# lh3/miniwfa

Hardware: AMD Instinct MI355X
Metric: aligned Gbp/s (q+t) (higher is better)
Workload: dtype int16x2 packed, range-guarded (bit-exact to the reference's int32); 1 GPU; 1024 pairs/GPU x 10000 bp, 0.05 divergence, score-only mwf_wfa_exact, default penalties (BASELINE configs[2]); pairs_this_gpu=1024, pairs_total=1024, target_len=10000, bases_this_gpu=20479492, grid=512, block=512

## Files before the change

### miniwfa_amd/build.py

```python
from __future__ import annotations

import os
import subprocess
import sys

HERE = os.path.dirname(os.path.abspath(__file__))
ROOT = os.path.dirname(HERE)
CSRC = os.path.join(HERE, "csrc")
LIB = os.path.join(CSRC, "libmwf_hip.so")
SOURCES = ["mwf_band2.hip", "mwf_band2_tab.hip", "mwf_band2_nib.hip", "mwf_band2_e3.hip", "mwf_band2_e4.hip", "mwf_band2_bi.hip", "mwf_band2_bi_deep.hip", "mwf_kernels.hip", "mwf_sketch.hip", "mwf_ends.hip", "mwf_lane.hip", "mwf_mid.hip", "mwf_sys.hip", "mwf_sys_deep.hip", "mwf_cigar_ops.hip", "mwf_cigar_text.hip", "mwf_alphabet.hip", "mwf_engine.cpp", "mwf_memory.cpp", "mwf_plan.cpp", "mwf_chain.cpp", "mwf_async.cpp", "kalloc.cpp", "mwf_dbg.cpp"]
HEADERS = [os.path.join(CSRC, "mwf_internal.h"), os.path.join(CSRC, "mwf_device.h"), os.path.join(CSRC, "mwf_ends.h"), os.path.join(CSRC, "mwf_sys_pass.h"), os.path.join(CSRC, "mwf_band2_kernel.h"), os.path.join(CSRC, "mwf_band2_dispatch.h"), os.path.join(CSRC, "mwf_engine.h"), os.path.join(CSRC, "mwf_plan_classes.h"), os.path.join(CSRC, "mwf_plan_retry.h"), os.path.join(ROOT, "include", "miniwfa.h"), os.path.join(ROOT, "include", "kalloc.h")]
BAND2_UNITS = [s for s in SOURCES if s.startswith("mwf_band2")]


def hipcc() -> str:
    for cand in (os.environ.get("HIPCC"), "/opt/rocm/bin/hipcc", "hipcc"):
        if cand and (os.path.isabs(cand) and os.path.exists(cand) or not os.path.isabs(cand)):
            return cand
    return "hipcc"


def stale() -> bool:
    if not os.path.exists(LIB):
        return True
    t = os.path.getmtime(LIB)
    deps = [os.path.join(CSRC, s) for s in SOURCES if os.path.exists(os.path.join(CSRC, s))] + HEADERS + [os.path.abspath(__file__)]
    return any(os.path.getmtime(d) > t for d in deps)


def build(force: bool = False, verbose: bool = False) -> str:
    if not force and not stale():
        return LIB
    from concurrent.futures import ThreadPoolExecutor
    objdir = os.path.join(CSRC, "build")
    os.makedirs(objdir, exist_ok=True)
    flags = ["--offload-arch=gfx950", "-O3", "-std=c++17", "-fPIC", "-Wall", "-Wno-unused-function", "-I", os.path.join(ROOT, "include"), "-I", CSRC]
    hdr_time = max(os.path.getmtime(h) for h in HEADERS + [os.path.abspath(__file__)])
    jobs, objs = [], []
    for name in SOURCES:
        src = os.path.join(CSRC, name)
        if not os.path.exists(src):
            continue
        obj = os.path.join(objdir, name + ".o")
        objs.append(obj)
        if force or not os.path.exists(obj) or os.path.getmtime(obj) < max(os.path.getmtime(src), hdr_time):
            jobs.append([hipcc(), *flags, "-c", src, "-o", obj])

    def run(cmd):
        if verbose:
            print(" ".join(cmd))
        return cmd, subprocess.run(cmd, capture_output=True, text=True)

    with ThreadPoolExecutor(max(1, min(8, len(jobs)))) as ex:
        for cmd, r in ex.map(run, jobs):
            if r.returncode != 0:
                sys.stderr.write(r.stdout + r.stderr)
                raise RuntimeError("hipcc failed: " + " ".join(cmd))
            if verbose and r.stderr.strip():
                sys.stderr.write(r.stderr)
    cmd, r = run([hipcc(), "--offload-arch=gfx950", "-fPIC", "-shared", *objs, "-o", LIB + ".tmp", "-lpthread"])
    if r.returncode != 0:
        sys.stderr.write(r.stdout + r.stderr)
        raise RuntimeError("hipcc failed linking libmwf_hip.so")
    os.replace(LIB + ".tmp", LIB)
    return LIB


KERNEL_FILES = {"wfa_band2_kernel": "mwf_band2_kernel.h", "wfa_band2_tab_kernel": "mwf_band2_kernel.h", "wfa_band2_nib_kernel": "mwf_band2_kernel.h", "wfa_sys_kernel": "mwf_sys.hip", "wfa_sys_seg_kernel": "mwf_sys.hip",
                "wfa_batch_kernel": "mwf_kernels.hip", "wfa_lane_kernel": "mwf_lane.hip", "wfa_mid_kernel": "mwf_mid.hip", "wfa_ends_kernel": "mwf_ends.hip"}
KERNEL_HEADERS = {"mwf_sys.hip": ["mwf_sys_pass.h", "mwf_sys_deep.hip"], "mwf_band2_kernel.h": ["mwf_band2_dispatch.h", *BAND2_UNITS]}


def kernel_fingerprint(symbol: str) -> str | None:
    import hashlib
    name = symbol.split("<")[0].strip()
    f = KERNEL_FILES.get(name)
    if f is None:
        return None
    h = hashlib.sha256()
    for p in [os.path.join(CSRC, x) for x in [f, *KERNEL_HEADERS.get(f, []), "mwf_device.h", "mwf_internal.h"]]:
        try:
            h.update(open(p, "rb").read())
        except OSError:
            return None
    return h.hexdigest()[:16]


CLI = os.path.join(ROOT, "tools", "test-mwf")


def build_cli(force: bool = False) -> str:
    src = os.path.join(ROOT, "tools", "test-mwf.cpp")
    if not force and os.path.exists(CLI) and os.path.getmtime(CLI) >= max(os.path.getmtime(src), os.path.getmtime(LIB)):
        return CLI
    zl = ["-DMWF_HAVE_ZLIB", "-lz"] if os.path.exists("/usr/include/zlib.h") else []
    cmd = ["g++", "-O2", "-std=c++17", "-Wall", "-I", os.path.join(ROOT, "include"), src, "-o", CLI,
           "-L", CSRC, "-lmwf_hip", "-Wl,-rpath," + CSRC] + zl
    r = subprocess.run(cmd, capture_output=True, text=True)
    if r.returncode != 0:
        sys.stderr.write(r.stdout + r.stderr)
        raise RuntimeError("g++ failed building tools/test-mwf")
    return CLI


if __name__ == "__main__":
    if "--list-band-units" in sys.argv or "--list-sources" in sys.argv:
        print(" ".join(BAND2_UNITS if "--list-band-units" in sys.argv else SOURCES))
        sys.exit(0)
    print(build(force="--force" in sys.argv, verbose=True))
    print(build_cli(force="--force" in sys.argv))
```

### miniwfa_amd/csrc/mwf_band2.hip

```cpp
#include "mwf_band2_dispatch.h"

namespace mwf {

namespace band2_text {
constexpr int kFoldMaxLag = 8;
constexpr int32_t kBiasOver = 1500, kBiasMargin = 600;
static_assert(kFoldMaxLag == mwf::kFoldMaxLag && kBiasOver == mwf::kBiasOver && kBiasMargin == mwf::kBiasMargin, "mwf_band2.hip: the copy of the kernel's constants is out of date");
}

namespace {
struct Unit {
	using Sets = MainSets;
	using BiasedSets = MainBiasedSets;
	static constexpr unsigned geos = kGeoBiased | kGeoPlain;
};
}

bool band2_supported(const Penalty &p)
{
	return (has_pen_set(MainSets{}, p.e1, p.e2) || has_pen_set(E3Sets{}, p.e1, p.e2) || has_pen_set(E4Sets{}, p.e1, p.e2)) && p.nH <= kMaxRing;
}

bool band2_biased512_supported(const Penalty &p)
{
	return has_pen_set(MainBiasedSets{}, p.e1, p.e2) || has_pen_set(BiSets{}, p.e1, p.e2) || has_pen_set(BiDeepSets{}, p.e1, p.e2);
}

int band2_span_chunks() { return kSpanT / 64 * kSpanK; }
int band2_biased512_chunks() { return 8 * kW4K; }

int launch_band2(const BatchArgs &a, int grid, const BandGeom &g0, void *stream)
{
	const int e1 = a.pen.e1;
	BandGeom g = g0;
	if (g.nib) return launch_band2_nib(a, grid, g, stream);
	if (g.tab > 0) {
		const int rc = launch_band2_tab(a, grid, g, stream);
		if (rc != -1) return rc;
		g.lds_bytes -= g.tab, g.tab = 0;
	}
	if (g.packed == 2 && !has_pen_set(MainBiasedSets{}, e1, a.pen.e2)) return e1 <= 2 ? launch_band2_bi1(a, grid, g, stream) : launch_band2_bi2(a, grid, g, stream);
	if (e1 == 3) return launch_band2_e3(a, grid, g, stream);
	if (e1 == 4) return launch_band2_e4(a, grid, g, stream);
	return band2_unit_launch<Unit>(a, grid, g, stream);
}

int band2_kernel_occupancy(const Penalty &p, const BandGeom &g, bool cigar)
{
	if (g.nib) return band2_occupancy_nib(p, g, cigar);
	if (g.tab > 0) return band2_occupancy_tab(p, g, cigar);
	if (g.packed == 2 && !has_pen_set(MainBiasedSets{}, p.e1, p.e2)) return p.e1 <= 2 ? band2_occupancy_bi1(p, g, cigar) : band2_occupancy_bi2(p, g, cigar);
	if (p.e1 == 3) return band2_occupancy_e3(p, g, cigar);
	if (p.e1 == 4) return band2_occupancy_e4(p, g, cigar);
	return band2_unit_occupancy<Unit>(p, g, cigar);
}

}
```

### miniwfa_amd/csrc/mwf_band2_dispatch.h

```cpp
#pragma once
#include "mwf_band2_kernel.h"

namespace mwf {

namespace {

template <int E1, int E2> struct PenSet { static constexpr int e1 = E1, e2 = E2; };
template <class... S> struct PenSets {};

template <class... S>
constexpr bool has_pen_set(PenSets<S...>, int e1, int e2) { return ((e1 == S::e1 && e2 == S::e2) || ...); }

template <class R, class F>
R for_pen_set(PenSets<>, int, int, R none, F &&) { return none; }
template <class R, class F, class S0, class... S>
R for_pen_set(PenSets<S0, S...>, int e1, int e2, R none, F &&f)
{
	if (e1 == S0::e1 && e2 == S0::e2) return f(S0{});
	return for_pen_set(PenSets<S...>{}, e1, e2, none, f);
}

#ifdef MWF_BAND_DEV
using MainSets = PenSets<PenSet<2, 1>>;
#else
using MainSets = PenSets<PenSet<2, 1>, PenSet<2, 2>, PenSet<1, 1>>;
#endif
using E3Sets = PenSets<PenSet<3, 1>, PenSet<3, 2>>;
using E4Sets = PenSets<PenSet<4, 1>>;
using MainBiasedSets = PenSets<PenSet<2, 1>>;
using BiSets = PenSets<PenSet<2, 2>, PenSet<1, 1>>;
using BiDeepSets = PenSets<PenSet<3, 1>, PenSet<3, 2>, PenSet<4, 1>>;
using TabSets = PenSets<PenSet<2, 1>>;
using NibSets = PenSets<PenSet<2, 1>>;
using NoSets = PenSets<>;

template <int T_, int K_, bool BI4_ = false> struct Geo { static constexpr int T = T_, K = K_; static constexpr bool BI4 = BI4_; };

inline bool geom_four_slots(const BandGeom &g) { return g.block == 512 && g.span > 512 / 64 * kWideK * kChunk; }
inline bool geom_five_slots(const BandGeom &g) { return geom_four_slots(g) && g.packed == 2; }
inline bool geom_six_slots(const BandGeom &g) { return g.block == 512 && g.span > 8 * kW4K * kChunk && g.packed == 2; }

enum : unsigned {
	kGeoBiased = 1,
	kGeoWide = 2,
	kGeoBytes = 4,
	kGeoSpan = 8,
#ifdef MWF_BAND_DEV
	kGeoSmall = 0,
#else
	kGeoSmall = 16,
#endif
	kGeoPlain = kGeoWide | kGeoBytes | kGeoSpan | kGeoSmall
};

template <unsigned GEOS, class R, class F>
R for_band_geom(const BandGeom &g, R none, F &&f)
{
	if constexpr ((GEOS & kGeoBiased) != 0) {
		if (geom_six_slots(g)) return f(Geo<512, kW4K + 1, true>{});
		if (geom_five_slots(g)) return f(Geo<512, kW4K, true>{});
	}
	if constexpr ((GEOS & kGeoWide) != 0) {
		if (geom_four_slots(g)) return f(Geo<512, 4>{});
		if (g.block == 512) return f(Geo<kWideT, kWideK>{});
	}
	if constexpr ((GEOS & kGeoBytes) != 0) {
		if (g.block == 768) return f(Geo<768, 2>{});
	}
	if constexpr ((GEOS & kGeoSpan) != 0) {
		if (g.block == kSpanT) return f(Geo<kSpanT, kSpanK>{});
	}
	if constexpr ((GEOS & kGeoSmall) != 0) {
		if (g.block == 256) return f(Geo<256, 3>{});
		if (g.block == 128) return f(Geo<128, 3>{});
		if (g.block == 64) return f(Geo<64, 3>{});
	}
	return none;
}

template <class U, class R, class F>
R band2_select(int e1, int e2, const BandGeom &g, R none, F &&f)
{
	return for_band_geom<U::geos>(g, none, [&](auto geo) {
		using Sets = std::conditional_t<decltype(geo)::BI4, typename U::BiasedSets, typename U::Sets>;
		return for_pen_set(Sets{}, e1, e2, none, [&](auto set) { return f(geo, set); });
	});
}

template <class U>
int band2_unit_launch(const BatchArgs &a, int grid, const BandGeom &g, void *stream)
{
	return band2_select<U>(a.pen.e1, a.pen.e2, g, -1, [&](auto geo, auto set) {
		using G = decltype(geo);
		using S = decltype(set);
		return launch_one<G::T, G::K, S::e1, S::e2, G::BI4>(a, grid, g.lds_bytes, g.tab, g.seq2 != 0, (hipStream_t)stream);
	});
}

template <class U>
int band2_unit_occupancy(const Penalty &p, const BandGeom &g, bool cigar)
{
	return band2_select<U>(p.e1, p.e2, g, 0, [&](auto geo, auto set) {
		using G = decltype(geo);
		using S = decltype(set);
		return occ_one<G::T, G::K, S::e1, S::e2, G::BI4>(g.lds_bytes, g.seq2 != 0, cigar);
	});
}

}

}
```

### miniwfa_amd/csrc/mwf_band2_kernel.h

```cpp
#pragma once
#include <cstddef>
#include <cstdio>
#include <cstdlib>
#include <type_traits>
#include "mwf_device.h"

#ifndef MWF_BAND2_FORM
#define MWF_BAND2_FORM 0
#endif
#if MWF_BAND2_FORM == 1
#define MWF_BAND2_KERNEL wfa_band2_tab_kernel
#elif MWF_BAND2_FORM == 2
#define MWF_BAND2_KERNEL wfa_band2_nib_kernel
#else
#define MWF_BAND2_KERNEL wfa_band2_kernel
#endif

namespace mwf {

using namespace dev;

namespace {

extern __shared__ __attribute__((aligned(16))) uint8_t lds2[];

constexpr int kWideT = 512, kWideK = 3;
constexpr int kWaves768 = 1;
constexpr int kSpanK = 5;
constexpr int kW4K = 5;
constexpr int kSpanT = 1024;
constexpr bool is_span(int T, int K) { return T == kSpanT && K == kSpanK; }
constexpr int kWideWaves = 4;
constexpr int kChunk = 256;
constexpr int kFoldMaxLag = 8;
constexpr int32_t kDeadPair = (int32_t)0x80008000u;
constexpr bool kTabProbe = MWF_BAND2_FORM == 1;
constexpr bool kNib = MWF_BAND2_FORM == 2;
constexpr int kSeqSh = kNib ? 2 : 1, kSeqDw = kNib ? 3 : 4, kSeqPer = 1 << kSeqDw;
constexpr uint32_t kNibTag = 0x40;
constexpr bool band2_geo_cached(int T, int K, bool TB) { return kTabProbe && T == 512 && (K == 3 || (K == 4 && !TB)); }
constexpr int kTabSlack = 258;

__device__ __forceinline__ int32_t lo16(int32_t v) { return (int32_t)(int16_t)(v & 0xffff); }
__device__ __forceinline__ int32_t hi16(int32_t v) { return v >> 16; }
__device__ __forceinline__ int32_t pack2(int32_t a, int32_t b)
{
	typedef short short2_t __attribute__((ext_vector_type(2)));
	const short2_t v = __builtin_amdgcn_cvt_pk_i16(a, b);
	return __builtin_bit_cast(int32_t, v);
}

__device__ __forceinline__ uint32_t seq4(int32_t off)
{
	const uint32_t *p = (const uint32_t*)(lds2 + (off & ~3));
	return __builtin_amdgcn_alignbyte(p[1], p[0], (uint32_t)off);
}

__device__ __forceinline__ int32_t lead_eq(uint32_t x)
{
	int32_t fb;
	asm("v_ffbl_b32 %0, %1" : "=v"(fb) : "v"(x));
	return (int32_t)((uint32_t)fb >> 3);
}

template <bool WANT_TB>
__device__ __forceinline__ Cell cell16(int32_t hx, int32_t o1m, int32_t g1m, int32_t o2m, int32_t g2m,
                                       int32_t o1p, int32_t g1p, int32_t o2p, int32_t g2p)
{
	if (!WANT_TB) return wf_cell<false>(hx, o1m, g1m, o2m, g2m, o1p, g1p, o2p, g2p);
	Cell c;
	c.e1 = max(o1m, g1m);
	c.e2 = max(o2m, g2m);
	c.f1 = max(o1p, g1p) + 1;
	c.f2 = max(o2p, g2p) + 1;
	const int32_t e = max(c.e1, c.e2), f = max(c.f1, c.f2), g = max(e, f), m = hx + 1;
	c.h = max(m, g);
	const uint32_t z = c.h == m ? 0u : c.h == c.e1 ? 1u : c.h == c.e2 ? 3u : c.h == c.f1 ? 2u : 4u;
	c.tb = z | ((uint32_t)(c.e1 != o1m) << 3) | ((uint32_t)(c.f1 != o1p + 1) << 4) | ((uint32_t)(c.e2 != o2m) << 5) | ((uint32_t)(c.f2 != o2p + 1) << 6);
	(void)e, (void)f, (void)g;
	return c;
}

struct Probe8 { uint32_t t0, t1, t2, q0, q1, q2; };
__device__ __forceinline__ void probe8_issue(Probe8 &p, int32_t j, int32_t aq)
{
	const uint32_t *pt = (const uint32_t*)(lds2 + (j & ~3)), *pq = (const uint32_t*)(lds2 + (aq & ~3));
	p.t0 = pt[0], p.t1 = pt[1], p.t2 = pt[2], p.q0 = pq[0], p.q1 = pq[1], p.q2 = pq[2];
}
__device__ __forceinline__ int32_t probe8_count(const Probe8 &p, int32_t j, int32_t aq)
{
	const uint32_t x0 = __builtin_amdgcn_alignbyte(p.t1, p.t0, (uint32_t)j) ^ __builtin_amdgcn_alignbyte(p.q1, p.q0, (uint32_t)aq);
	const uint32_t x1 = __builtin_amdgcn_alignbyte(p.t2, p.t1, (uint32_t)j) ^ __builtin_amdgcn_alignbyte(p.q2, p.q1, (uint32_t)aq);
	return min(min(lead_eq(x0), lead_eq(x1) + 4), 9);
}

__device__ __forceinline__ uint32_t seq16(int32_t base, int32_t j)
{
	const uint32_t *p = (const uint32_t*)(lds2 + base + ((j >> kSeqDw) << 2));
	return __builtin_amdgcn_alignbit(p[1], p[0], (uint32_t)j << kSeqSh);
}
__device__ __forceinline__ int32_t lead_eq2(uint32_t x)
{
	int32_t fb;
	asm("v_ffbl_b32 %0, %1" : "=v"(fb) : "v"(x));
	return (int32_t)((uint32_t)fb >> kSeqSh);
}
struct Probe16 { uint32_t t0, t1, q0, q1; };
__device__ __forceinline__ void probe16_issue(Probe16 &p, int32_t qbase, int32_t j, int32_t iq)
{
	const uint32_t *pt = (const uint32_t*)(lds2 + ((j >> 4) << 2)), *pq = (const uint32_t*)(lds2 + qbase + ((iq >> 4) << 2));
	p.t0 = pt[0], p.t1 = pt[1], p.q0 = pq[0], p.q1 = pq[1];
}
__device__ __forceinline__ int32_t probe16_count(const Probe16 &p, int32_t j, int32_t iq)
{
	return min(lead_eq2(__builtin_amdgcn_alignbit(p.t1, p.t0, (uint32_t)j << 1) ^ __builtin_amdgcn_alignbit(p.q1, p.q0, (uint32_t)iq << 1)), 17);
}
__device__ __forceinline__ int32_t run_wave16(int32_t qbase, int32_t j, int32_t iq, int32_t room, int32_t n0, int32_t tbase = 0)
{
	const int32_t lane = threadIdx.x & 63;
	int32_t n = n0;
	while (n < room) {
		const int32_t off = n + kSeqPer * lane;
		int32_t m = 0;
		if (off < room) m = min(min(lead_eq2(seq16(tbase, j + off) ^ seq16(qbase, iq + off)), kSeqPer), room - off);
		const unsigned long long stop = __ballot(m < kSeqPer);
		if (stop == 0) { n += 64 * kSeqPer; continue; }
		const int32_t first = (int32_t)__builtin_ctzll(stop);
		n += kSeqPer * first + __builtin_amdgcn_readlane(m, first);
		break;
	}
	return min(n, room);
}
template <int T>
__device__ __forceinline__ uint32_t pack2bit(const uint8_t *src, int32_t len, int32_t base)
{
	uint32_t bad = 0;
	const int32_t n_dw = (len >> 4) + 2;
	for (int32_t w = threadIdx.x; w < n_dw; w += T) {
		uint32_t out = 0;
		const int32_t b0 = w << 4;
		if (b0 + 16 <= len) {
			uint32_t q[4];
			__builtin_memcpy(q, src + b0, 16);
#pragma unroll
			for (int k = 0; k < 4; ++k) {
				const uint32_t x = q[k], code = (x >> 1) & 0x03030303u;
				const uint32_t lo1 = code & 0x01010101u, hi1 = (code >> 1) & 0x01010101u;
				const uint32_t expect = 0x41414141u + (lo1 & ~hi1) * 0x02u + (hi1 & ~lo1) * 0x13u + (hi1 & lo1) * 0x06u;
				bad |= x ^ expect;
				out |= ((code | code >> 6 | code >> 12 | code >> 18) & 0xffu) << (8 * k);
			}
		} else {
#pragma unroll 1
			for (int32_t k = 0; k < 16 && b0 + k < len; ++k) {
				const uint32_t x = src[b0 + k], code = (x >> 1) & 3u;
				bad |= x ^ ((0x47544341u >> (8 * code)) & 0xffu);
				out |= code << (2 * k);
			}
		}
		*(uint32_t*)(lds2 + base + 4 * w) = out;
	}
	return bad;
}

template <int T>
__device__ __forceinline__ uint32_t pack4bit(const uint8_t *src, int32_t len, int32_t base)
{
	uint32_t bad = 0;
	const int32_t n_dw = (len >> 3) + 2;
	for (int32_t w = 2 * (int32_t)threadIdx.x; w < n_dw; w += 2 * T) {
		uint32_t out[2] = {0, 0};
		const int32_t b0 = w << 3;
		if (b0 + 16 <= len) {
			uint32_t q[4];
			__builtin_memcpy(q, src + b0, 16);
#pragma unroll
			for (int k = 0; k < 4; ++k) {
				const uint32_t x = q[k];
				bad |= (x & 0xf0f0f0f0u) ^ (kNibTag * 0x01010101u);
				uint32_t c = x & 0x0f0f0f0fu;
				c = (c | c >> 4) & 0x00ff00ffu;
				c = (c | c >> 8) & 0xffffu;
				out[k >> 1] |= c << (16 * (k & 1));
			}
		} else {
#pragma unroll 1
			for (int32_t k = 0; k < 16 && b0 + k < len; ++k) {
				const uint32_t x = src[b0 + k];
				bad |= (x & 0xf0u) ^ kNibTag;
				out[k >> 3] |= (x & 0xfu) << (4 * (k & 7));
			}
		}
		*(uint32_t*)(lds2 + base + 4 * w) = out[0];
		if (w + 1 < n_dw) *(uint32_t*)(lds2 + base + 4 * w + 4) = out[1];
	}
	return bad;
}

template <int T>
__device__ __forceinline__ void build_probe_table(int32_t tl, int32_t ql, int32_t tbase, int32_t qbase)
{
	const int32_t n = tl + ql + kTabSlack;
	for (int32_t e = threadIdx.x; e < n; e += T) {
		const int32_t q = e - tl - 2;
		uint32_t v = 0;
		if (e <= tl) v = seq16(tbase, e);
		else if (q >= 0 && q <= ql) v = seq16(qbase, q);
		*(uint16_t*)(lds2 + 2 * e) = (uint16_t)v;
	}
}

__device__ __forceinline__ unsigned long long lane_mask(int32_t base, int32_t k, int32_t a, int32_t b)
{
	int32_t lmin = a - base - k, lmax = b - base - k;
	if (lmax < 0) return 0ull;
	lmin = lmin <= 0 ? 0 : (lmin + 3) >> 2;
	lmax = min(lmax >> 2, 63);
	if (lmin > lmax) return 0ull;
	return (~0ull >> (63 - lmax)) & (~0ull << lmin);
}

__device__ __forceinline__ int32_t run_wave2(int32_t j, int32_t aq, int32_t room, int32_t n0)
{
	const int32_t lane = threadIdx.x & 63;
	int32_t n = n0;
	while (n < room) {
		const int32_t off = n + 4 * lane;
		int32_t m = 0;
		if (off < room) {
			const uint32_t x = seq4(j + off) ^ seq4(aq + off);
			m = min(min(lead_eq(x), 4), room - off);
		}
		const unsigned long long stop = __ballot(m < 4);
		if (stop == 0) { n += 256; continue; }
		const int32_t first = (int32_t)__builtin_ctzll(stop);
		n += 4 * first + __builtin_amdgcn_readlane(m, first);
		break;
	}
	return min(n, room);
}

constexpr int32_t kBiasOver = 1500, kBiasMargin = 600;
__device__ __forceinline__ int32_t wide_bias(int32_t tl) { return max(tl + kBiasOver - 32767, 0); }

template <int D, int NWK>
struct alignas(16) Band2Lds {
	Shared sh;
	int32_t edge[D][NWK + 2][4];
	int32_t dump[64 * 2 + (2 * NWK + 4) * 4];
};

typedef short s16x2 __attribute__((ext_vector_type(2)));
__device__ __forceinline__ int32_t pk_max(int32_t a, int32_t b) { return MWF_BC(int32_t, __builtin_elementwise_max(MWF_BC(s16x2, a), MWF_BC(s16x2, b))); }
__device__ __forceinline__ int32_t pk_add(int32_t a, int32_t b) { return MWF_BC(int32_t, (s16x2)(MWF_BC(s16x2, a) + MWF_BC(s16x2, b))); }
__device__ __forceinline__ int32_t pk_sub(int32_t a, int32_t b) { return MWF_BC(int32_t, (s16x2)(MWF_BC(s16x2, a) - MWF_BC(s16x2, b))); }
__device__ __forceinline__ int32_t bfi(int32_t mask, int32_t a, int32_t b) { return (a & mask) | (b & ~mask); }
__device__ __forceinline__ int32_t half_of(int32_t v, int hi) { return hi ? v >> 16 : (int32_t)(int16_t)(v & 0xffff); }
__device__ __forceinline__ int32_t pair_of(int32_t lo, int32_t hi) { return (int32_t)(((uint32_t)hi << 16) | ((uint32_t)lo & 0xffffu)); }

__device__ __forceinline__ int32_t left_of_A(int32_t B, int32_t fill) { return __builtin_amdgcn_alignbit(B, from_left(B, fill), 16); }
__device__ __forceinline__ int32_t right_of_B(int32_t A, int32_t fill) { return __builtin_amdgcn_alignbit(from_right(A, fill), A, 16); }

template <int T, int K, int E1, int E2, bool TB, bool S2, bool BI4, bool FOLD, typename ArgsT>
__device__ PassResult band2_pass(const ArgsT &A, const PairMem &M, Shared &sh, const int32_t edge_base, const int32_t qoff, bool trace_band)
{
	constexpr int NW = T / 64, NWK = NW * K, D = (E1 > E2 ? E1 : E2) + 1;
	constexpr bool BI = is_span(T, K) || BI4;
	constexpr bool TAB = kTabProbe && S2;
	constexpr int FULL = TAB ? 8 : S2 ? kSeqPer : 8;
	constexpr bool kChain = TAB;
	constexpr bool kGeo = TAB && band2_geo_cached(T, K, TB);
#define MWF_RARE(x) (kChain ? __builtin_expect((x), 0) != 0 : (x))
	constexpr int kAgeOut = FOLD ? kFoldMaxLag : D;
	constexpr int kAge = (NWK + 2) * 16;
	static_assert(D >= 2 && D <= 5, "edge-table ages");
	const int32_t tl = M.tl, ql = M.ql, cmax = tl + ql + 1;
	const int32_t tid = threadIdx.x, lane = tid & 63, wave = uni(tid >> 6);
	const int32_t W = A.W, nH = A.pen.nH, lagx = A.pen.x, lag1 = A.pen.oe1, lag2 = A.pen.oe2;
	const int32_t B = BI ? wide_bias(tl) : 0;
	const int32_t ONEB = BI ? both16(1 + B) : 0x00010001;
	char *const Hb = (char*)M.H;
	const uint32_t RS = (uint32_t)W << 1;
	const int32_t min_lag = min(lagx, min(lag1, lag2));
	const bool relaxed_stores = min_lag >= 3;
	PassResult R;
	R.status = ST_OK, R.s = 0, R.info = 0, R.n_snap = 0, R.cells = 0;

	static_assert(E1 >= 1 && E1 <= 4 && (E2 == 1 || E2 == 2), "history depth");
	int32_t e1h[E1][K][2], f1h[E1][K][2], e2h[E2][K][2], f2h[E2][K][2];
#pragma unroll
	for (int k = 0; k < K; ++k)
#pragma unroll
		for (int i = 0; i < 2; ++i) {
#pragma unroll
			for (int a = 0; a < E1; ++a) e1h[a][k][i] = f1h[a][k][i] = kDeadPair;
#pragma unroll
			for (int a = 0; a < E2; ++a) e2h[a][k][i] = f2h[a][k][i] = kDeadPair;
		}
	const int32_t RA = pair_of(4 * lane, 4 * lane + 2);
	const uint32_t lane8 = ((uint32_t)lane << 3) + 8u;
	const int32_t nd = lane == 0 ? -4 : 8;
	const int32_t T0 = both16(cmax), TLp = both16(tl), TL1 = both16(tl + 1);
	const int32_t ebase = edge_base + wave * 16, dump_base = edge_base + D * kAge + NW * 16;
	const int32_t dump_lane = dump_base + lane * 8;
	int32_t epos[D];
#pragma unroll
	for (int a = 0; a < D; ++a) epos[a] = a * kAge;

	{
		const int32_t reach = nH + 1 + 8, g_a = max(tl + 1 - reach, 0) >> 8, n_g = ((tl + 1 + reach) >> 8) - g_a + 1, per_row = n_g * 64;
		for (int32_t q = tid; q < nH * per_row; q += T) {
			const int32_t row = q / per_row, rem = q - row * per_row;
			*(int2*)(Hb + (size_t)((uint32_t)row * RS + (uint32_t)(g_a * 512 + rem * 8 + 8))) = make_int2(kDeadPair, kDeadPair);
		}
	}
	for (int32_t j = tid; j < D * (NWK + 2) * 4; j += T) *(int32_t*)(lds2 + edge_base + 4 * j) = kDeadPair;
	if (tid == 0) {
		for (int32_t j = 0; j < nH; ++j) sh.rng_lo[j] = 1, sh.rng_hi[j] = 0;
		for (int32_t j = 0; j < 12; ++j) (&sh.flags[0][0])[j] = 0;
		sh.rng_lo[0] = sh.rng_hi[0] = tl + 1;
		sh.word[3] = -1;
	}
	__syncthreads();
	if (tid < 64) {
		const int32_t k0 = (S2 ? run_wave16(qoff, 0, 0, min(tl, ql), 0, TAB ? fresh(A).band_lds_tab : 0) : run_wave2(0, qoff, min(tl, ql), 0)) - 1;
		if (tid == 0) {
			const int32_t c = tl + 1, e = c & 3;
			*(int16_t*)(Hb + 8 + (size_t)(uint32_t)(((c & ~3) + ((e & 1) << 1) + (e >> 1)) << 1)) = (int16_t)(k0 - B);
			sh.word[1] = k0;
		}
	}
	__syncthreads();
	{
		const int32_t k0 = uni(sh.word[1]);
		if (k0 == tl - 1 && k0 == ql - 1) return R;
	}

	int32_t s = 0, wf_lo = tl + 1, wf_hi = tl + 1;
	int32_t curH = 0, par = 0;
	const uint32_t ring_bytes = (uint32_t)nH * RS;
	uint32_t bn = (uint32_t)(1 % nH) * RS, bx = (uint32_t)((nH - lagx + 1) % nH) * RS, b1 = (uint32_t)((nH - lag1 + 1) % nH) * RS, b2 = (uint32_t)((nH - lag2 + 1) % nH) * RS;
	struct Rows { int2 HX, O1, O2; int32_t N1, N2; } pre;
	pre.HX = pre.O1 = pre.O2 = make_int2(0, 0), pre.N1 = pre.N2 = 0;
	auto load_rows = [&](Rows &r, const char *rx, const char *r1, const char *r2, uint32_t off) {
		const uint32_t noff = off + (uint32_t)nd;
		r.HX = *(const int2*)(rx + off), r.O2 = *(const int2*)(r2 + off);
		r.N2 = *(const int32_t*)(r2 + noff);
		if (!FOLD) r.O1 = *(const int2*)(r1 + off), r.N1 = *(const int32_t*)(r1 + noff);
	};
	const int64_t iter_limit = A.max_iter > 0 ? A.max_iter : INT64_MAX;
	int64_t cells = kChain ? iter_limit : 0, tb_used = 0;
	int32_t est_window = 0;
	const int32_t s_limit = A.max_s > 0 ? A.max_s : INT32_MAX;
	const int64_t rows_slot = TB ? A.rows_slot : 0, tb_slot_bytes = TB ? A.tb_slot_bytes : 0;

	int32_t gl = (wf_lo > 1 ? wf_lo - 1 : 1) >> 8, gk[K];
	int32_t grjA[K], grjB[K], gdA[K];
	auto remap = [&](int32_t g_lo) {
		const int32_t base = g_lo - g_lo % NWK;
#pragma unroll
		for (int k = 0; k < K; ++k) {
			int32_t g = base + wave + NW * k;
			if (g < g_lo) g += NWK;
			gk[k] = g;
			if (kGeo) {
				const int32_t cbp = both16(g * kChunk), xAc = pk_subsat(pk_subsat(T0, cbp), RA);
				grjA[k] = pk_minu(xAc, TLp), grjB[k] = pk_minu(pk_subsat(xAc, 0x00010001), TLp);
				gdA[k] = pk_add(pk_add(RA, cbp), 0x00010001);
			}
		}
	};
	remap(gl);
	int32_t idle[K];
#pragma unroll
	for (int k = 0; k < K; ++k) idle[k] = kAgeOut;
	int32_t up_wait = 0, up_min = 0;
	int32_t ekey = 0;
	constexpr bool kEpoch = !is_span(T, K) && T != 64;
	uint32_t est = 0;
	static_assert(kEpoch || ((NW & (NW - 1)) == 0 && !(T == 512 && K == 4)), "the full header of the gated geometries is written for a power-of-two wave count and no three-slot note");
	static_assert(K <= 6, "slot classes of the window epoch: four bits per slot below bit 24");
	constexpr bool kLeanTail = kChain;
	static_assert(!kLeanTail || (kEpoch && K <= 4), "the table form keeps one more bit per slot in est, from bit 26 on");
	constexpr uint32_t kRunBits = 0x111111u & ((1u << (4 * K)) - 1u);

	auto step = [&]() __attribute__((always_inline)) -> bool {
		constexpr int P1 = E1 - 1, P2 = E2 - 1;
#ifdef MWF_B2_TIMING
		const uint64_t tm0 = __builtin_readcyclecounter();
#endif
		const int32_t lo = wf_lo > 1 ? wf_lo - 1 : 1;
		const int32_t hi = wf_hi < cmax ? wf_hi + 1 : cmax;
		const int32_t lo_p = lo, hi_p = hi;
		const int32_t s_new = s + 1;
		const int32_t newH = curH + 1 == nH ? 0 : curH + 1;
		const int32_t npar = par + 1 == 3 ? 0 : par + 1;
		const int32_t origin = lo & ~3;
		const int32_t row_bytes = (hi | 3) - origin + 1;
		if (TB) {
			if (s_new - 1 >= rows_slot) { R.status = ST_ROWS_OVERFLOW; return true; }
			if (tb_used + row_bytes > tb_slot_bytes) { R.status = ST_TB_OVERFLOW; return true; }
		}
		const int32_t gl_next = (lo > 1 ? lo - 1 : 1) >> 8;
		const int32_t ga = lo >> 8, gb = hi >> 8;
		const int32_t key = gl_next | gb << 15 | 1 << 29 | (ga - gl_next) << 30;
		const bool fast = kEpoch && key == ekey;
		uint32_t st = est;
		bool act[K];
		if (!kEpoch) {
			if (gb - min(ga, gl + 1) + 3 > NWK - 1)
				if (((hi < cmax ? hi + 1 : cmax) >> 8) - min(gl_next, gl) + 1 > NWK - 1) { R.status = ST_BAND_OVERFLOW; return true; }
			if (BI && cmax - lo > 65535) { R.status = ST_BAND_OVERFLOW; return true; }
		} else if (!fast) {
			bool hold = true;
			if (gb - min(ga, gl + 1) + 3 > NWK - 1) {
				if (((hi < cmax ? hi + 1 : cmax) >> 8) - min(gl_next, gl) + 1 > NWK - 1) { R.status = ST_BAND_OVERFLOW; return true; }
				hold = false;
			}
			if (T == 512 && K == 4 && R.n_snap == 0 && gb - ga + 3 > 23) {
				if (((hi < cmax ? hi + 1 : cmax) >> 8) - gl_next + 1 > 23) R.n_snap = 1;
				hold = false;
			}
			if (BI) {
				if (cmax - lo > 65535) { R.status = ST_BAND_OVERFLOW; return true; }
				if (cmax - (ga << 8) > 65535) hold = false;
			}
			const int32_t gspan = gb - ga;
			int n_busy = 0;
			st = 0;
#pragma unroll
			for (int k = 0; k < K; ++k) {
				if ((uint32_t)(gk[k] - ga) <= (uint32_t)gspan) {
					idle[k] = 0;
					st |= (1u | (gk[k] == ga ? 2u : 0u) | (gk[k] == gb ? 4u : 0u)) << (4 * k);
					if (kLeanTail && (uint32_t)(ql + 1 - gk[k] * kChunk) < (uint32_t)kChunk) st |= 1u << (26 + k);
					if (k < 2 || k == K - 1) ++n_busy;
				} else if (idle[k] < kAgeOut) {
					++idle[k];
					st |= 9u << (4 * k);
					hold = false;
				}
			}
			if ((NW & (NW - 1)) == 0) {
				const int32_t pos = (wave - ga) & (NW - 1);
				const int32_t left = gspan + 1 - pos + ((pos == 0 || ((gb - wave) & (NW - 1)) == 0) ? NW : 0);
				if (left > 2 * NW) __builtin_amdgcn_s_setprio(3);
				else if (left > NW) __builtin_amdgcn_s_setprio(2);
				else if (left > 0) __builtin_amdgcn_s_setprio(1);
				else __builtin_amdgcn_s_setprio(0);
			} else {
				if (n_busy >= 3) __builtin_amdgcn_s_setprio(3);
				else if (n_busy == 2) __builtin_amdgcn_s_setprio(2);
				else if (n_busy == 1) __builtin_amdgcn_s_setprio(1);
				else __builtin_amdgcn_s_setprio(0);
			}
			if (ga >= 1 && wave == (ga - 1) % NW) st |= 1u << 24;
			if (wave == (gb + 1) % NW) st |= 1u << 25;
			est = st, ekey = kEpoch && hold ? ~key : -1;
		}
		const char *const rowx = Hb + bx, *const row1 = Hb + b1, *const row2 = Hb + b2;
		char *const rown = Hb + bn;
		const bool track_good = (((256 - (s_new & 255)) & 255) < nH);
		const int32_t rE1 = ebase + epos[E1 - 1], rE2 = ebase + epos[E2 - 1];
		const int32_t wE = lane == 63 ? ebase + epos[D - 1] : dump_lane, wF = lane == 0 ? ebase + epos[D - 1] : dump_lane;
		auto put_edge = [&](int k, int32_t e1b, int32_t e2b, int32_t f1a, int32_t f2a) {
			*(int2*)(lds2 + wE + (k * NW + 1) * 16) = make_int2(e1b, e2b);
			*(int2*)(lds2 + wF + (k * NW + 1) * 16 + 8) = make_int2(f1a, f2a);
			if (k == K - 1 && wave == NW - 1) *(int2*)(lds2 + wE - (NW - 1) * 16) = make_int2(e1b, e2b);
			if (k == 0 && wave == 0) *(int2*)(lds2 + wF + (NWK + 1) * 16 + 8) = make_int2(f1a, f2a);
		};
		const bool forecast = NWK < 24 ? (s_new == 64 || s_new == 256 || s_new == 1024) : NWK >= 64 ? (s_new == 1024 || s_new == 4096) : false;
		int32_t far = kDeadPair;
		const int32_t cfin = ql + 1;

		if (wave == 0) {
			sh.rng_lo[newH] = lo, sh.rng_hi[newH] = hi;
			sh.flags[npar + 1 == 3 ? 0 : npar + 1][0] = 0;
			if (TB) M.row_off[s_new - 1] = tb_used, M.row_lo[s_new - 1] = origin;
#ifndef MWF_B2_TIMING
			if (trace_band && s_new - 1 < fresh(A).dbg_cap) M.dbg[2 * (s_new - 1)] = lo, M.dbg[2 * (s_new - 1) + 1] = hi;
#endif
		}

		if (!kEpoch) {
#pragma unroll
			for (int k = 0; k < K; ++k) act[k] = (uint32_t)(gk[k] - ga) <= (uint32_t)(gb - ga);
			const int32_t pos = (wave - ga) & (NW - 1);
			const int32_t left = gb - ga + 1 - pos + ((pos == 0 || ((gb - wave) & (NW - 1)) == 0) ? NW : 0);
			if (left > 2 * NW) __builtin_amdgcn_s_setprio(3);
			else if (left > NW) __builtin_amdgcn_s_setprio(2);
			else if (left > 0) __builtin_amdgcn_s_setprio(1);
			else __builtin_amdgcn_s_setprio(0);
		}
#ifdef MWF_B2_TIMING
		int n_act = 0;
#pragma unroll
		for (int k = 0; k < K; ++k) n_act += (kEpoch ? (st >> (4 * k) & 9u) == 1u : act[k]) ? 1 : 0;
#endif

#ifdef MWF_B2_TIMING
		const uint64_t tm1 = __builtin_readcyclecounter();
#endif
		int n_stores = 0;
		if (kEpoch ? (st & (1u << 24)) != 0 : (ga >= 1 && wave == (ga - 1) % NW)) *(int2*)(rown + ((uint32_t)((ga - 1) << 9) + lane8)) = make_int2(kDeadPair, kDeadPair);
		if (kEpoch ? (st & (1u << 25)) != 0 : wave == (gb + 1) % NW) *(int2*)(rown + ((uint32_t)((gb + 1) << 9) + lane8)) = make_int2(kDeadPair, kDeadPair);
#if MWF_B2_TIMING == 2
#ifndef MWF_B2_TIMED_CHUNK
#define MWF_B2_TIMED_CHUNK 0
#endif
		int chunks_seen = 0;
		uint32_t ct[4] = {0, 0, 0, 0};
#endif
#pragma unroll
		for (int k = 0; k < K; ++k) {
			const uint32_t cls = st >> (4 * k);
			if (kEpoch) {
				if (!(cls & 1u)) continue;
			} else if (!act[k]) {
				if (idle[k] >= kAgeOut) continue;
				++idle[k];
			} else idle[k] = 0;
			const bool edgy = (cls & 0xeu) != 0;
			int32_t lo = uni(lo_p), hi = uni(hi_p);
			asm volatile("" : "+s"(lo), "+s"(hi));
			const int32_t g = gk[k], cb = g * kChunk, c0 = cb + 4 * lane;
#if MWF_B2_TIMING == 2
			uint64_t tc0 = 0, tc1 = 0, tc2 = 0, tc3 = 0, tc4 = 0;
			const bool timed = chunks_seen++ == MWF_B2_TIMED_CHUNK;
			if (timed) asm volatile("s_memtime %0\n\ts_waitcnt lgkmcnt(0)" : "=s"(tc0) :: "memory");
#endif
			const uint32_t off = (uint32_t)(cb << 1) + lane8;
			load_rows(pre, rowx, row1, row2, off);
			const int2 HX = pre.HX, O1 = pre.O1, O2 = pre.O2;
			const int32_t N1 = pre.N1, N2 = pre.N2;
			const int32_t xE1 = *(const int32_t*)(lds2 + rE1 + k * NW * 16), xE2 = *(const int32_t*)(lds2 + rE2 + k * NW * 16 + 4);
			const int32_t xF1 = *(const int32_t*)(lds2 + rE1 + (k * NW + 2) * 16 + 8), xF2 = *(const int32_t*)(lds2 + rE2 + (k * NW + 2) * 16 + 12);
			const bool inside = (kEpoch && !edgy) || (cb >= lo && cb + kChunk - 1 <= hi);

			const int32_t E1a = e1h[P1][k][0], E1b = e1h[P1][k][1], F1a = f1h[P1][k][0], F1b = f1h[P1][k][1];
			const int32_t E2a = e2h[P2][k][0], E2b = e2h[P2][k][1], F2a = f2h[P2][k][0], F2b = f2h[P2][k][1];
			const int32_t o1mA = FOLD ? 0 : left_of_A(O1.y, N1), o2mA = left_of_A(O2.y, N2), g1mA = left_of_A(E1b, xE1), g2mA = left_of_A(E2b, xE2);
			const int32_t o1pB = FOLD ? 0 : right_of_B(O1.x, N1), o2pB = right_of_B(O2.x, N2), g1pB = right_of_B(F1a, xF1), g2pB = right_of_B(F2a, xF2);
			const int32_t ONE = 0x00010001;
			int32_t ne1A = FOLD ? g1mA : pk_max(o1mA, g1mA), ne2A = pk_max(o2mA, g2mA);
			int32_t ne1B = FOLD ? E1a : pk_max(O1.x, E1a), ne2B = pk_max(O2.x, E2a);
			const int32_t pf1A = FOLD ? F1b : pk_max(O1.y, F1b), pf2A = pk_max(O2.y, F2b);
			const int32_t pf1B = FOLD ? g1pB : pk_max(o1pB, g1pB), pf2B = pk_max(o2pB, g2pB);
			int32_t nf1A = pk_add(pf1A, ONE), nf2A = pk_add(pf2A, ONE), nf1B = pk_add(pf1B, ONE), nf2B = pk_add(pf2B, ONE);
			const int32_t mA = pk_add(HX.x, ONE), mB = pk_add(HX.y, ONE);
			int32_t hA, hB;
			if (kChain) {
				const int32_t gA = pk_max(mA, pk_max(ne1A, ne2A)), gB = pk_max(mB, pk_max(ne1B, ne2B)), fA = pk_max(nf1A, nf2A), fB = pk_max(nf1B, nf2B);
				__builtin_amdgcn_sched_group_barrier(0x2, 1, 0);
				hA = pk_max(gA, fA), hB = pk_max(gB, fB);
			} else {
				hA = pk_max(pk_max(mA, pk_max(ne1A, ne2A)), pk_max(nf1A, nf2A));
				hB = pk_max(pk_max(mB, pk_max(ne1B, ne2B)), pk_max(nf1B, nf2B));
			}
#if MWF_B2_TIMING == 2
			if (timed) asm volatile("s_memtime %0\n\ts_waitcnt lgkmcnt(0)" : "=s"(tc1) : "v"(hA), "v"(hB) : "memory");
#endif
			uint32_t tbw = 0;
			if (TB) {
				const int32_t TWO = 0x00020002, NEG1 = (int32_t)0xffffffffu, EIGHT = 0x00080008, C16 = 0x00100010, C32 = 0x00200020, C64 = 0x00400040;
				int32_t zA = pk_mad(pk_ne1(hA, nf1A), TWO, NEG1), zB = pk_mad(pk_ne1(hB, nf1B), TWO, NEG1);
				zA = pk_mad(pk_ne1(hA, ne2A), zA, TWO), zB = pk_mad(pk_ne1(hB, ne2B), zB, TWO);
				zA = pk_mad(pk_ne1(hA, ne1A), zA, ONE), zB = pk_mad(pk_ne1(hB, ne1B), zB, ONE);
				zA = pk_mad(pk_ne1(hA, mA), zA, 0), zB = pk_mad(pk_ne1(hB, mB), zB, 0);
				if (!FOLD) {
					zA = pk_mad(pk_ne1(ne1A, o1mA), EIGHT, zA), zB = pk_mad(pk_ne1(ne1B, O1.x), EIGHT, zB);
					zA = pk_mad(pk_ne1(pf1A, O1.y), C16, zA), zB = pk_mad(pk_ne1(pf1B, o1pB), C16, zB);
				}
				zA = pk_mad(pk_ne1(ne2A, o2mA), C32, zA), zB = pk_mad(pk_ne1(ne2B, O2.x), C32, zB);
				zA = pk_mad(pk_ne1(pf2A, O2.y), C64, zA), zB = pk_mad(pk_ne1(pf2B, o2pB), C64, zB);
				tbw = (uint32_t)zA | ((uint32_t)zB << 8);
			}
			const int32_t cbp = both16(cb);
			const int32_t xA = pk_sub(pk_sub(T0, cbp), RA);
			const int32_t xAc = TAB ? pk_subsat(pk_subsat(T0, cbp), RA) : xA;
			const int32_t rjA = kGeo ? grjA[k] : pk_minu(xAc, TLp), rjB = kGeo ? grjB[k] : pk_minu(TAB ? pk_subsat(xAc, ONE) : pk_sub(xA, ONE), TLp);
			const int32_t dA = kGeo ? gdA[k] : TAB ? pk_add(pk_add(RA, cbp), ONE) : pk_sub(pk_add(RA, cbp), TL1), dB = pk_add(dA, ONE);
			const bool on_lo = kEpoch ? (cls & 2u) != 0 : g == ga, on_hi = kEpoch ? (cls & 4u) != 0 : g == gb;
			const bool special = is_span(T, K) || (BI4 && !TB) || (kEpoch ? edgy : !inside || on_lo || on_hi) || track_good;
			int32_t outA = 0, outB = 0;
			uint32_t bits = 0, gbits = 0;
			if (MWF_RARE(special)) {
			if (MWF_RARE(!inside)) {
				const int32_t lo_r = both16(min(max(lo - cb, 0), 256)), hi_r1 = both16(min(max(hi - cb + 1, 0), 256));
				const int32_t RB = pk_add(RA, 0x00010001), RB1 = pk_add(RA, 0x00020002);
				outA = pk_nonzero_mask(pk_subsat(lo_r, RA) | pk_subsat(RB, hi_r1));
				outB = pk_nonzero_mask(pk_subsat(lo_r, RB) | pk_subsat(RB1, hi_r1));
				hA = bfi(outA, kDeadPair, hA), hB = bfi(outB, kDeadPair, hB);
				ne1A = bfi(outA, kDeadPair, ne1A), ne1B = bfi(outB, kDeadPair, ne1B);
				ne2A = bfi(outA, kDeadPair, ne2A), ne2B = bfi(outB, kDeadPair, ne2B);
				nf1A = bfi(outA, kDeadPair, nf1A), nf1B = bfi(outB, kDeadPair, nf1B);
				nf2A = bfi(outA, kDeadPair, nf2A), nf2B = bfi(outB, kDeadPair, nf2B);
			}
			if (on_lo || on_hi) {
				if (on_lo) {
					const int32_t rel = lo - cb;
					const int32_t v = half_of(__builtin_amdgcn_readlane((rel & 1) ? hB : hA, rel >> 2), (rel >> 1) & 1);
					bits |= v >= -1 - B ? 1u : 0u;
				}
				if (on_hi) {
					const int32_t rel = hi - cb;
					const int32_t v = half_of(__builtin_amdgcn_readlane((rel & 1) ? hB : hA, rel >> 2), (rel >> 1) & 1);
					bits |= v >= -1 - B ? 2u : 0u;
				}
			}
			if (track_good) {
				auto bad = [&](int32_t v, int32_t rj) { return pk_subsat(pk_add(v, ONEB), rj); };
				const int32_t bA = pk_minu(pk_minu(bad(hA, rjA), pk_minu(bad(ne1A, rjA), bad(nf1A, rjA))), pk_minu(bad(ne2A, rjA), bad(nf2A, rjA))) | outA;
				const int32_t bB = pk_minu(pk_minu(bad(hB, rjB), pk_minu(bad(ne1B, rjB), bad(nf1B, rjB))), pk_minu(bad(ne2B, rjB), bad(nf2B, rjB))) | outB;
				gbits = (uint32_t)((bA & 0xffff) == 0) | (uint32_t)((bB & 0xffff) == 0) << 1 | (uint32_t)(((uint32_t)bA >> 16) == 0) << 2 | (uint32_t)(((uint32_t)bB >> 16) == 0) << 3;
				if (BI && (s_new & 255) == 0) {
					const int32_t width = both16(kBiasMargin), from = both16(-1 - B - kBiasMargin), top = both16(32768 - kBiasMargin);
					auto stray = [&](int32_t v, int32_t lo_end) { return pk_subsat(width, pk_sub(v, lo_end)); };
					const int32_t any = stray(hA, from) | stray(hB, from) | stray(ne1A, from) | stray(ne1B, from) | stray(ne2A, from) | stray(ne2B, from) |
					                    stray(nf1A, from) | stray(nf1B, from) | stray(nf2A, from) | stray(nf2B, from) | stray(hA, top) | stray(hB, top);
					if (__ballot(any != 0)) bits |= 0x80u;
				}
			}
			if (kLeanTail && bits != 0 && lane == 0) atomicOr((unsigned int*)&sh.flags[npar][0], bits);
			}
			if (FOLD) {
				ne1A = pk_max(ne1A, HX.x), ne1B = pk_max(ne1B, HX.y), nf1A = pk_max(nf1A, HX.x), nf1B = pk_max(nf1B, HX.y);
				if (TB) {
					const int32_t EIGHT = 0x00080008, C16 = 0x00100010;
					const int32_t fA = pk_mad(pk_ne1(ne1A, HX.x), EIGHT, pk_mad(pk_ne1(nf1A, HX.x), C16, 0));
					const int32_t fB = pk_mad(pk_ne1(ne1B, HX.y), EIGHT, pk_mad(pk_ne1(nf1B, HX.y), C16, 0));
					tbw |= (uint32_t)fA | ((uint32_t)fB << 8);
				}
			}
			e1h[P1][k][0] = ne1A, e1h[P1][k][1] = ne1B, f1h[P1][k][0] = nf1A, f1h[P1][k][1] = nf1B;
			e2h[P2][k][0] = ne2A, e2h[P2][k][1] = ne2B, f2h[P2][k][0] = nf2A, f2h[P2][k][1] = nf2B;
#pragma unroll
			for (int i = 0; i < 2; ++i) {
#pragma unroll
				for (int a = E1 - 1; a > 0; --a) {
					asm volatile("v_swap_b32 %0, %1" : "+v"(e1h[a - 1][k][i]), "+v"(e1h[a][k][i]));
					asm volatile("v_swap_b32 %0, %1" : "+v"(f1h[a - 1][k][i]), "+v"(f1h[a][k][i]));
				}
#pragma unroll
				for (int a = E2 - 1; a > 0; --a) {
					asm volatile("v_swap_b32 %0, %1" : "+v"(e2h[a - 1][k][i]), "+v"(e2h[a][k][i]));
					asm volatile("v_swap_b32 %0, %1" : "+v"(f2h[a - 1][k][i]), "+v"(f2h[a][k][i]));
				}
			}
			put_edge(k, ne1B, ne2B, nf1A, nf2A);

#if MWF_B2_TIMING == 2
			if (timed) asm volatile("s_memtime %0\n\ts_waitcnt lgkmcnt(0)" : "=s"(tc2) : "v"(hA), "v"(hB), "v"(rjA), "v"(dA) : "memory");
#endif
			const int32_t jA = pk_minu(pk_add(hA, ONEB), rjA), jB = pk_minu(pk_add(hB, ONEB), rjB);
			const int32_t iqA = pk_add(jA, dA), iqB = pk_add(jB, dB);
			int32_t cnt[4];
			if (TAB) {
				uint32_t tv[4], qv[4];
#pragma unroll
				for (int u = 0; u < 4; ++u) {
					const uint32_t J = (uint32_t)((u & 1) ? jB : jA), Q = (uint32_t)((u & 1) ? iqB : iqA);
					uint32_t ta, qa;
					if (u & 2) {
						asm("v_add_u32_sdwa %0, %1, %1 dst_sel:DWORD dst_unused:UNUSED_PAD src0_sel:WORD_1 src1_sel:WORD_1" : "=v"(ta) : "v"(J));
						asm("v_add_u32_sdwa %0, %1, %1 dst_sel:DWORD dst_unused:UNUSED_PAD src0_sel:WORD_1 src1_sel:WORD_1" : "=v"(qa) : "v"(Q));
					} else {
						asm("v_add_u32_sdwa %0, %1, %1 dst_sel:DWORD dst_unused:UNUSED_PAD src0_sel:WORD_0 src1_sel:WORD_0" : "=v"(ta) : "v"(J));
						asm("v_add_u32_sdwa %0, %1, %1 dst_sel:DWORD dst_unused:UNUSED_PAD src0_sel:WORD_0 src1_sel:WORD_0" : "=v"(qa) : "v"(Q));
					}
					asm volatile("ds_read_u16 %0, %1" : "=v"(tv[u]) : "v"(ta));
					asm volatile("ds_read_u16 %0, %1" : "=v"(qv[u]) : "v"(qa));
				}
				asm volatile("s_waitcnt lgkmcnt(0)" : "+v"(tv[0]), "+v"(tv[1]), "+v"(tv[2]), "+v"(tv[3]), "+v"(qv[0]), "+v"(qv[1]), "+v"(qv[2]), "+v"(qv[3]));
#pragma unroll
				for (int u = 0; u < 4; ++u) asm("v_ffbl_b32 %0, %1" : "=v"(cnt[u]) : "v"(tv[u] ^ qv[u]));
			} else if (S2) {
				uint64_t tw[4], qw[4];
#pragma unroll
				for (int u = 0; u < 4; ++u) {
					const uint32_t J = (uint32_t)((u & 1) ? jB : jA), Q = (uint32_t)((u & 1) ? iqB : iqA);
					const uint32_t ta = kNib ? ((u & 2) ? (J >> 17) & 0x7ffcu : (J >> 1) & 0x7ffcu) : (u & 2) ? (J >> 18) & 0x3ffcu : (J >> 2) & 0x3ffcu;
					const uint32_t qa = (kNib ? ((u & 2) ? (Q >> 19) : ((Q >> 3) & 0x1fffu)) : ((u & 2) ? (Q >> 20) : ((Q >> 4) & 0xfffu))) * 4u + (uint32_t)qoff;
					asm volatile("ds_read2_b32 %0, %1 offset1:1" : "=v"(tw[u]) : "v"(ta));
					asm volatile("ds_read2_b32 %0, %1 offset1:1" : "=v"(qw[u]) : "v"(qa));
				}
				asm volatile("s_waitcnt lgkmcnt(0)" : "+v"(tw[0]), "+v"(tw[1]), "+v"(tw[2]), "+v"(tw[3]), "+v"(qw[0]), "+v"(qw[1]), "+v"(qw[2]), "+v"(qw[3]));
#pragma unroll
				for (int u = 0; u < 4; ++u) {
					const uint32_t J = (uint32_t)((u & 1) ? jB : jA), Q = (uint32_t)((u & 1) ? iqB : iqA);
					const uint32_t tsh = kNib ? ((u & 2) ? (J >> 14) & 28u : J << 2) : (u & 2) ? (BI ? (J >> 15) & 30u : J >> 15) : J << 1;
					const uint32_t qsh = kNib ? ((u & 2) ? (Q >> 14) & 28u : Q << 2) : (u & 2) ? (Q >> 15) & 30u : Q << 1;
					cnt[u] = lead_eq2(__builtin_amdgcn_alignbit((uint32_t)(tw[u] >> 32), (uint32_t)tw[u], tsh) ^ __builtin_amdgcn_alignbit((uint32_t)(qw[u] >> 32), (uint32_t)qw[u], qsh));
				}
			} else {
				constexpr int PF = (K >= 3 && T >= 512) ? 1 : 2;
#pragma unroll
				for (int h2 = 0; h2 < 4 / PF; ++h2) {
					Probe8 pr[PF];
					int32_t jj[PF], aq[PF];
#pragma unroll
					for (int v = 0; v < PF; ++v) {
						const int u = PF * h2 + v;
						jj[v] = (int32_t)((uint32_t)((u & 1) ? jB : jA) >> ((u & 2) ? 16 : 0) & 0xffffu);
						aq[v] = (int32_t)((uint32_t)((u & 1) ? iqB : iqA) >> ((u & 2) ? 16 : 0) & 0xffffu) + qoff;
						probe8_issue(pr[v], jj[v], aq[v]);
					}
#pragma unroll
					for (int v = 0; v < PF; ++v) cnt[PF * h2 + v] = probe8_count(pr[v], jj[v], aq[v]);
				}
			}
			typedef unsigned short us2_t __attribute__((ext_vector_type(2)));
			int32_t cA = MWF_BC(int32_t, (us2_t)__builtin_amdgcn_cvt_pk_u16((uint32_t)cnt[0], (uint32_t)cnt[2]));
			int32_t cB = MWF_BC(int32_t, (us2_t)__builtin_amdgcn_cvt_pk_u16((uint32_t)cnt[1], (uint32_t)cnt[3]));
			if (TAB) cA = MWF_BC(int32_t, (us2_t)(MWF_BC(us2_t, cA) >> 1)), cB = MWF_BC(int32_t, (us2_t)(MWF_BC(us2_t, cB) >> 1));
#if MWF_B2_TIMING == 2
			if (timed) asm volatile("s_memtime %0\n\ts_waitcnt lgkmcnt(0)" : "=s"(tc3) : "v"(cA), "v"(cB) : "memory");
#endif
			const int32_t FULLp = both16(FULL);
			const int32_t m9A = pk_minu(cA, pk_sub(rjA, jA)), m9B = pk_minu(cB, pk_sub(rjB, jB));
			int32_t nmA = pk_minu(m9A, FULLp), nmB = pk_minu(m9B, FULLp);
			const int32_t pendp = pk_subsat(m9A, FULLp) | pk_subsat(m9B, FULLp);
			if (MWF_RARE(__ballot(pendp != 0) != 0)) {
				const int32_t tb0 = TAB ? fresh(A).band_lds_tab : 0;
				int32_t hv[4] = {half_of(hA, 0) + B, half_of(hB, 0) + B, half_of(hA, 1) + B, half_of(hB, 1) + B};
				int32_t nmat[4] = {(int32_t)((uint32_t)nmA & 0xffffu), (int32_t)((uint32_t)nmB & 0xffffu), (int32_t)((uint32_t)nmA >> 16), (int32_t)((uint32_t)nmB >> 16)};
				const uint32_t pend = (uint32_t)(((uint32_t)m9A & 0xffffu) > (uint32_t)FULL) | (uint32_t)(((uint32_t)m9B & 0xffffu) > (uint32_t)FULL) << 1 |
				                      (uint32_t)(((uint32_t)m9A >> 16) > (uint32_t)FULL) << 2 | (uint32_t)(((uint32_t)m9B >> 16) > (uint32_t)FULL) << 3;
				uint32_t open = 0;
#pragma unroll
				for (int i = 0; i < 4; ++i) {
					if (__ballot((pend >> i) & 1u) == 0) continue;
					if ((pend >> i) & 1u) {
						int32_t n = FULL;
						const int32_t j = hv[i] + 1, q = c0 + i - 1 - tl + j, rm = min(tl - j, ql - q), aqq = qoff + q;
						for (int trip = 0; n < rm; ++trip) {
							if (trip == 4) { open |= 1u << i; break; }
							if (S2) {
								const int32_t m = min(lead_eq2(seq16(tb0, j + n) ^ seq16(qoff, q + n)), kSeqPer);
								n += m;
								if (m < kSeqPer) break;
							} else {
								const uint32_t xa = seq4(j + n) ^ seq4(aqq + n), xb = seq4(j + n + 4) ^ seq4(aqq + n + 4);
								if (xa | xb) { n += xa ? min(lead_eq(xa), 4) : 4 + min(lead_eq(xb), 4); break; }
								n += 8;
							}
						}
						nmat[i] = min(n, rm);
					}
				}
				for (unsigned long long owners = __ballot(open != 0); owners; owners &= owners - 1) {
					const int32_t src = (int32_t)__builtin_ctzll(owners);
					const int32_t c0s = cb + 4 * src;
					const uint32_t ob = (uint32_t)__builtin_amdgcn_readlane((int32_t)open, src);
#pragma unroll
					for (int i = 0; i < 4; ++i) {
						if (!((ob >> i) & 1u)) continue;
						const int32_t hh = __builtin_amdgcn_readlane(hv[i], src);
						const int32_t j = hh + 1, q = c0s + i - 1 - tl + j, rm = min(tl - j, ql - q);
						const int32_t n = S2 ? run_wave16(qoff, j, q, rm, FULL + 4 * kSeqPer, tb0) : run_wave2(j, qoff + q, rm, 40);
						nmat[i] = lane == src ? n : nmat[i];
					}
				}
				nmA = pair_of(nmat[0], nmat[2]), nmB = pair_of(nmat[1], nmat[3]);
			}
			const int32_t hxA = pk_add(hA, nmA), hxB = pk_add(hB, nmB);
			if (forecast) far = pk_max(far, pk_max(hxA, hxB));
			unsigned long long fm = 0;
			int32_t done_info = 0;
			bool end_bit = false;
			if constexpr (kLeanTail) end_bit = MWF_RARE((st & (1u << (26 + k))) != 0) && cfin >= lo && cfin <= hi;
			if (MWF_RARE(kLeanTail ? end_bit : (uint32_t)(cfin - cb) < (uint32_t)kChunk && cfin >= lo && cfin <= hi)) {
				const int32_t rel = cfin - cb, hi_half = (rel >> 1) & 1;
				const int32_t hv = half_of((rel & 1) ? hxB : hxA, hi_half) + B, nm = (int32_t)((uint32_t)((rel & 1) ? nmB : nmA) >> (hi_half ? 16 : 0) & 0xffffu);
				const uint32_t f = (uint32_t)(lane == (rel >> 2)) & (uint32_t)(hv == tl - 1) & inm_bit(ql - tl, hv - nm, tl, ql);
				done_info = (f && nm == 0) ? (int32_t)((tbw >> (8 * (rel & 3))) & 7u) : 0;
				fm = __ballot(f != 0);
				if (kLeanTail && fm) {
					const uint32_t fin = 4u | (uint32_t)__builtin_amdgcn_readlane(done_info, (int32_t)__builtin_ctzll(fm)) << 4;
					if (lane == 0) atomicOr((unsigned int*)&sh.flags[npar][0], fin);
				}
			}
			*(int2*)(rown + off) = make_int2(hxA, hxB);
			if (!kLeanTail) ++n_stores;
#if MWF_B2_TIMING == 2
			if (timed) {
				asm volatile("s_memtime %0\n\ts_waitcnt lgkmcnt(0)" : "=s"(tc4) : "v"(hxA), "v"(hxB) : "memory");
				ct[0] = (uint32_t)min(tc1 - tc0, (uint64_t)4095), ct[1] = (uint32_t)min(tc2 - tc1, (uint64_t)4095);
				ct[2] = (uint32_t)min(tc3 - tc2, (uint64_t)4095), ct[3] = (uint32_t)min(tc4 - tc3, (uint64_t)4095);
			}
#endif
			if (TB && c0 >= origin && c0 <= hi) *(uint32_t*)(M.tb + tb_used - origin + c0) = tbw;
			if (MWF_RARE(track_good)) {
				unsigned long long *gword = M.good + (int64_t)newH * fresh(A).GW + g * 4;
#pragma unroll
				for (int i = 0; i < 4; ++i) {
					const unsigned long long m = __ballot((gbits >> i) & 1u);
					if (lane == 0) gword[i] = m;
				}
			}
			if (!kLeanTail) {
				if (fm) bits |= 4u | (uint32_t)__builtin_amdgcn_readlane(done_info, (int32_t)__builtin_ctzll(fm)) << 4;
				if (kChain) {
					if (MWF_RARE(bits != 0))
						if (lane == 0) atomicOr((unsigned int*)&sh.flags[npar][0], bits);
				} else if (bits && lane == 0) atomicOr((unsigned int*)&sh.flags[npar][0], bits);
			}
		}

		if (forecast) {
			const int32_t m = wave_max(max(lo16(far), hi16(far))) + B;
			if (lane == 0 && m >= 0) atomicMax(&sh.word[3], m);
		}
#ifdef MWF_B2_TIMING
		const uint64_t tm2 = __builtin_readcyclecounter();
#endif
		if constexpr (!kChain) {
			bn = bn + RS == ring_bytes ? 0u : bn + RS, bx = bx + RS == ring_bytes ? 0u : bx + RS;
			b1 = b1 + RS == ring_bytes ? 0u : b1 + RS, b2 = b2 + RS == ring_bytes ? 0u : b2 + RS;
		}
		const bool young_store = relaxed_stores && (kLeanTail ? (st & kRunBits) != 0 : n_stores > 0) && !TB && !track_good;
		if (young_store) asm volatile("s_waitcnt vmcnt(1) lgkmcnt(0)" ::: "memory");
		else asm volatile("s_waitcnt vmcnt(0) lgkmcnt(0)" ::: "memory");
#ifdef MWF_B2_TIMING
		const uint64_t tm3 = __builtin_readcyclecounter();
#endif
		__builtin_amdgcn_s_barrier();
		asm volatile("" ::: "memory");

		uint32_t fl = 0;
		int32_t flv = 0;
		if constexpr (kChain) {
			static_assert(!kChain || !BI, "the range checks of the biased offsets leave before the penalty turns");
			asm volatile("ds_read_b32 %0, %1" : "=v"(flv) : "v"((uint32_t)(uintptr_t)&sh.flags[npar][0]) : "memory");
			bn = bn + RS == ring_bytes ? 0u : bn + RS, bx = bx + RS == ring_bytes ? 0u : bx + RS;
			b1 = b1 + RS == ring_bytes ? 0u : b1 + RS, b2 = b2 + RS == ring_bytes ? 0u : b2 + RS;
		} else fl = (uint32_t)uni(sh.flags[npar][0]);
#ifdef MWF_B2_TIMING
		if (trace_band && tid == (fresh(A).max_iter < 0 ? (int32_t)-fresh(A).max_iter : 0) && s_new - 1 < fresh(A).dbg_cap) {
			const uint64_t tm4 = __builtin_readcyclecounter();
#if MWF_B2_TIMING == 2
			M.dbg[2 * (s_new - 1)] = (int32_t)(ct[0] | ct[1] << 12 | (uint32_t)n_act << 28);
			M.dbg[2 * (s_new - 1) + 1] = (int32_t)(ct[2] | ct[3] << 12);
			(void)tm4;
#else
			M.dbg[2 * (s_new - 1)] = (int32_t)(min((uint32_t)(tm1 - tm0), 65535u) | min((uint32_t)(tm2 - tm1), 65535u) << 16);
			M.dbg[2 * (s_new - 1) + 1] = (int32_t)(min((uint32_t)(tm3 - tm2), 4095u) | min((uint32_t)(tm4 - tm3), 65535u) << 12 | (uint32_t)n_act << 28);
#endif
		}
#endif
		int32_t done = 0, payload = 0;
		if constexpr (!kChain) {
			if (fl & 1u) wf_lo = lo;
			if (fl & 2u) wf_hi = hi;
			done = (int32_t)((fl >> 2) & 1u), payload = (int32_t)((fl >> 4) & 7u);
			if (BI && (fl & 0x80u)) { R.status = ST_BAND_OVERFLOW; return true; }
		}
		s = s_new, curH = newH, par = npar;
		{
			const int32_t oldest = epos[D - 1];
#pragma unroll
			for (int a = D - 1; a > 0; --a) epos[a] = epos[a - 1];
			epos[0] = oldest;
		}
		if (!kEpoch || ekey < 0) {
			if (gl_next < gl) gl = gl_next, remap(gl), up_wait = 0, ekey = 0;
			else if (gl_next > gl) {
				up_min = up_wait == 0 ? gl_next : min(up_min, gl_next);
				if (++up_wait > kAgeOut) gl = up_min, remap(gl), up_wait = 0;
				ekey = 0;
			} else up_wait = 0, ekey = ~ekey;
		}
		if (TB) tb_used += row_bytes;
		if constexpr (kChain) {
			asm volatile("s_waitcnt lgkmcnt(0)" : "+v"(flv));
			fl = (uint32_t)__builtin_amdgcn_readfirstlane(flv);
			if (fl & 1u) wf_lo = lo;
			if (fl & 2u) wf_hi = hi;
			done = (int32_t)((fl >> 2) & 1u), payload = (int32_t)((fl >> 4) & 7u);
		}
		if ((s & 0xff) == 0) {
			if (tid == 0) sh.red[0] = 0x7fffffff, sh.red[1] = -1;
			__syncthreads();
			const int32_t gfirst = wf_lo >> 8, n_words = ((wf_hi >> 8) - gfirst + 1) * 4, GWc = fresh(A).GW;
			for (int32_t q = tid; q < n_words; q += T) {
				const int32_t gg = gfirst + (q >> 2), kq = q & 3, base = gg * kChunk;
				unsigned long long m = 0;
				for (int32_t j = 0; j < nH; ++j)
					if (sh.rng_lo[j] <= sh.rng_hi[j] && sh.rng_lo[j] <= base + kChunk - 1 && sh.rng_hi[j] >= base) m |= M.good[(int64_t)j * GWc + gg * 4 + kq];
				m &= lane_mask(base, kq, wf_lo, wf_hi);
				if (m) {
					atomicMin(&sh.red[0], base + 4 * (int32_t)__builtin_ctzll(m) + kq);
					atomicMax(&sh.red[1], base + 4 * (63 - (int32_t)__builtin_clzll(m)) + kq);
				}
			}
			__syncthreads();
			const int32_t glo = uni(sh.red[0]), ghi = uni(sh.red[1]);
			if (ghi < 0) { R.status = ST_INTERNAL; return true; }
			wf_lo = glo, wf_hi = ghi;
		}
		if (kChain) cells -= hi - lo + 1;
		else cells += hi - lo + 1;
		if ((kChain ? cells < 0 : cells > iter_limit) || s > s_limit) {
			R.status = ST_STOPPED;
			return true;
		}
		if (done) {
			R.info = payload;
			return true;
		}
		if (forecast) {
			est_window = window_forecast(s, uni(sh.word[3]), tl, ql, (NWK - 1) * kChunk - 64, NWK >= 24 && NWK < 64);
			if (est_window) { R.status = ST_BAND_OVERFLOW; return true; }
		}
		return false;
	};
	for (;;)
		if (step()) break;
	asm volatile("s_waitcnt vmcnt(0)" ::: "memory");
	if (kChain) cells = (fresh(A).max_iter > 0 ? fresh(A).max_iter : INT64_MAX) - cells;
	R.s = s, R.cells = est_window ? -(int64_t)est_window : cells;
	return R;
}
#undef MWF_RARE

constexpr int band2_waves(int T, int K, bool TB)
{
	return is_span(T, K) ? (T == 1024 ? 4 : 3) : T == 1024 ? 4 : T == kWideT ? kWideWaves : T <= 512 ? ((TB && T < 512) ? 3 : 4) : kWaves768;
}
template <int T, int K, int E1, int E2, bool TB, bool S2, bool BI4 = false, bool FOLD = false>
__global__ __launch_bounds__(T, band2_waves(T, K, TB)) void MWF_BAND2_KERNEL(const BatchArgs)
{
	constexpr int NWK = (T / 64) * K, D = (E1 > E2 ? E1 : E2) + 1;
	KArgs &A0 = kernel_args();
	if ((uint32_t)(uintptr_t)lds2 != 0u) __builtin_trap();
	typedef Band2Lds<D, NWK> LdsT;
	const int32_t lds_seq = A0.band_lds_seq;
	LdsT *const L = (LdsT*)(lds2 + lds_seq);
	Shared &sh = L->sh;
	const int32_t edge_base = lds_seq + (int32_t)offsetof(LdsT, edge);
	CigLocal cig_loc;
	cig_loc.base = 0, cig_loc.left = 0;
	for (int32_t round = 0;; ++round) {
		KArgs &A = fresh(A0);
		if (threadIdx.x == 0) sh.item = A.queue ? (int32_t)atomicAdd(A.queue, 1) : (round == 0 ? (int32_t)blockIdx.x : A.n_pairs), sh.word[2] = 0;
		__syncthreads();
		const int32_t item = uni(sh.item);
		__syncthreads();
		if (item >= A.n_pairs) break;
		const int32_t pair = A.order ? A.order[item] : item;
		PairMem M;
		pair_mem(A, (int32_t)blockIdx.x, pair, M);
		constexpr bool TAB = kTabProbe && S2;
		const int32_t toff = TAB ? A.band_lds_tab : 0;
		const int32_t qoff = toff + (S2 ? ((M.tl >> kSeqDw) + 2) * 4 : ((M.tl + 3) & ~3) + 8);
		PassResult R;
		R.status = ST_OK, R.s = 0, R.info = 0, R.n_snap = 0, R.cells = 0;
		if (S2) {
			uint32_t bad = kNib ? pack4bit<T>(M.ts, M.tl, toff) : pack2bit<T>(M.ts, M.tl, toff);
			bad |= kNib ? pack4bit<T>(M.qs, M.ql, qoff) : pack2bit<T>(M.qs, M.ql, qoff);
			if (bad) sh.word[2] = 1;
			__syncthreads();
			if (uni(sh.word[2])) R.status = ST_ALPHABET;
			if (TAB) {
				if (2 * (M.tl + M.ql + kTabSlack) > toff) R.status = ST_BAND_OVERFLOW;
				else if (R.status == ST_OK) build_probe_table<T>(M.tl, M.ql, toff, qoff);
			}
		} else {
			for (int32_t j = threadIdx.x; j < M.tl; j += T) lds2[j] = M.ts[j];
			for (int32_t j = threadIdx.x; j < M.ql; j += T) lds2[qoff + j] = M.qs[j];
			__syncthreads();
		}
		const bool trace = A.dbg && pair == A.debug_pair;
		if (R.status == ST_OK) R = band2_pass<T, K, E1, E2, TB, S2, BI4, FOLD>(A, M, sh, edge_base, qoff, trace);
		if (T == 512 && K == 4 && R.n_snap && threadIdx.x == 0 && fresh(A0).report_wide) atomicOr((unsigned int*)(fresh(A0).cig_head + 1), 1u);
		R.n_snap = 0;
		if (S2 && !kNib) M.t2 = lds2 + toff, M.q2 = lds2 + qoff;
		if (TB && FOLD) M.tb_fwd = 1;
		finish_pair(fresh(A0), M, (int32_t)blockIdx.x, pair, R, R.status, 0, T <= 256 ? &cig_loc : nullptr);
	}
}

template <int T, int K, int E1, int E2>
constexpr int lds_tail() { return (int)sizeof(Band2Lds<(E1 > E2 ? E1 : E2) + 1, (T / 64) * K>); }

inline bool band2_folds(const Penalty &p, bool band_fold) { return band_fold && p.oe1 - p.x == p.e1 && p.oe1 < kFoldMaxLag; }
constexpr bool band2_has_folded(int T, int E1, bool TB, bool S2) { return T >= 512 && S2 && E1 == 2 && !(kNib && TB); }
constexpr bool kFoldedOnly = kTabProbe;

template <int T, int K, int E1, int E2, bool TB, bool S2, bool BI4, bool FOLD>
void launch_kernel(const BatchArgs &a, int grid, int lds, hipStream_t st)
{
	if (lds > 48 * 1024) {
		(void)hipFuncSetAttribute(reinterpret_cast<const void*>(&MWF_BAND2_KERNEL<T, K, E1, E2, TB, S2, BI4, FOLD>), hipFuncAttributeMaxDynamicSharedMemorySize, lds);
		(void)hipGetLastError();
	}
	if (getenv("MWF_DEBUG")) {
		if (kNib)
			fprintf(stderr, "[libmwf_hip] band2 nib launch: wfa_band2_nib_kernel T %d K %d E1 %d E2 %d TB %d S2 %d BI4 %d FOLD %d, %d pairs, grid %d, lds %d B\n", T, K, E1, E2, (int)TB, (int)S2, (int)BI4, (int)FOLD, (int)a.n_pairs, grid, lds);
		else
			fprintf(stderr, "[libmwf_hip] band2 launch: T %d K %d E1 %d E2 %d TB %d S2 %d BI4 %d FOLD %d, %d pairs, grid %d\n", T, K, E1, E2, (int)TB, (int)S2, (int)BI4, (int)FOLD, (int)a.n_pairs, grid);
		if (kTabProbe) fprintf(stderr, "[libmwf_hip] band2 table probe: table %d B, lds %d B\n", (int)a.band_lds_tab, lds);
	}
	hipLaunchKernelGGL((MWF_BAND2_KERNEL<T, K, E1, E2, TB, S2, BI4, FOLD>), dim3(grid), dim3(T), lds, st, a);
}

template <int T, int K, int E1, int E2, bool TB, bool S2, bool BI4 = false>
void launch_variant(const BatchArgs &a, int grid, int lds, hipStream_t st)
{
	if constexpr (kFoldedOnly) return launch_kernel<T, K, E1, E2, TB, S2, BI4, true>(a, grid, lds, st);
	else {
		if constexpr (band2_has_folded(T, E1, TB, S2)) {
			if (band2_folds(a.pen, a.band_fold)) return launch_kernel<T, K, E1, E2, TB, S2, BI4, true>(a, grid, lds, st);
		}
		launch_kernel<T, K, E1, E2, TB, S2, BI4, false>(a, grid, lds, st);
	}
}

template <int T, int K, int E1, int E2, bool TB, bool S2, bool BI4 = false>
int occ_variant(int lds)
{
	int n = 0;
	return hipOccupancyMaxActiveBlocksPerMultiprocessor(&n, MWF_BAND2_KERNEL<T, K, E1, E2, TB, S2, BI4, kFoldedOnly>, T, lds) == hipSuccess ? n : 0;
}

constexpr bool band2_geo_seq2(int T) { return T != 768; }

template <int T, int K, int E1, int E2, bool BI4 = false>
int launch_one(const BatchArgs &a0, int grid, int lds_seq, int lds_tab, bool seq2, hipStream_t st)
{
	constexpr bool S2 = band2_geo_seq2(T);
	if (seq2 != S2) return -1;
	BatchArgs a = a0;
	a.band_lds_seq = lds_seq, a.band_lds_tab = lds_tab;
	const int lds = lds_seq + lds_tail<T, K, E1, E2>();
	if (a.want_cigar) launch_variant<T, K, E1, E2, true, S2, BI4>(a, grid, lds, st);
	else launch_variant<T, K, E1, E2, false, S2, BI4>(a, grid, lds, st);
	return hipGetLastError() == hipSuccess ? 0 : -2;
}

template <int T, int K, int E1, int E2, bool BI4 = false>
int occ_one(int lds_seq, bool seq2, bool tb)
{
	constexpr bool S2 = band2_geo_seq2(T);
	if (seq2 != S2) return 0;
	const int lds = lds_seq + lds_tail<T, K, E1, E2>();
	return tb ? occ_variant<T, K, E1, E2, true, S2, BI4>(lds) : occ_variant<T, K, E1, E2, false, S2, BI4>(lds);
}

}

}
```

### miniwfa_amd/csrc/mwf_engine.cpp

```cpp
#include "mwf_engine.h"

extern "C" {


int mwf_gpu_device_count(void)
{
	int n = 0;
	if (hipGetDeviceCount(&n) != hipSuccess) { (void)hipGetLastError(); return 0; }
	return n;
}

mwf_gpu_t *mwf_gpu_create(int device, void *stream)
{
	int n = mwf_gpu_device_count();
	if (device < 0 || device >= n) return nullptr;
	if (hipSetDevice(device) != hipSuccess) return nullptr;
	mwf_gpu_t *g = new mwf_gpu_t();
	g->device = device;
	hipDeviceProp_t prop;
	if (hipGetDeviceProperties(&prop, device) != hipSuccess) { delete g; return nullptr; }
	g->n_cu = prop.multiProcessorCount;
	g->total_mem = prop.totalGlobalMem;
	if (stream) g->stream = (hipStream_t)stream;
	else {
		if (hipStreamCreateWithFlags(&g->stream, hipStreamNonBlocking) != hipSuccess) { delete g; return nullptr; }
		g->own_stream = true;
	}
	(void)hipEventCreate(&g->ev0);
	(void)hipEventCreate(&g->ev1);
	if (ensure(g, g->queue, kQueueInts * 4) || hipMemsetAsync(g->queue.p, 0, kQueueInts * 4, g->stream) != hipSuccess) {
		mwf_gpu_destroy(g);
		return nullptr;
	}
	return g;
}

static void trim(mwf_gpu_t *g)
{
	(void)hipStreamSynchronize(g->stream);
	for (DevBuf *b : {&g->ring, &g->sring, &g->good, &g->tb, &g->row_off, &g->row_lo, &g->cig_scratch, &g->snap, &g->snap_meta, &g->seg, &g->dbg,
	                  &g->coop_misc, &g->sys_box, &g->sys_prog, &g->sys_log, &g->sys_ep, &g->sys_park, &g->sys_ring, &g->sys_sring, &g->sys_good, &g->retry_ids,
	                  &g->spare_block, &g->spare_cig})
		release(g, *b);
	g->dev_bytes_peak = g->dev_bytes;
}

void mwf_gpu_destroy(mwf_gpu_t *g)
{
	if (!g) return;
	(void)hipSetDevice(g->device);
	trim(g);
	release(g, g->queue);
	if (g->pin) (void)hipHostFree(g->pin);
	if (g->res_pin) (void)hipHostFree(g->res_pin);
	for (hipEvent_t e : {g->ev0, g->ev1, g->pin_ev[0], g->pin_ev[1], g->ev_alpha[0], g->ev_alpha[1], g->ev_alpha[2], g->ev_alpha[3]})
		if (e) (void)hipEventDestroy(e);
	if (g->own_stream) (void)hipStreamDestroy(g->stream);
	delete g;
}

const char *mwf_gpu_last_error(const mwf_gpu_t *g) { return g ? g->err.c_str() : "no engine (no gfx950 device could be opened)"; }

int mwf_gpu_set(mwf_gpu_t *g, const char *name, int64_t value)
{
	if (!g || !name) return -1;
	if (!strcmp(name, "tb_budget_mb")) g->tb_budget_mb = value;
	else if (!strcmp(name, "lowmem_budget_mb")) g->lowmem_budget_mb = std::max<int64_t>(0, value);
	else if (!strcmp(name, "coop_min_len")) g->coop_min_len = value;
	else if (!strcmp(name, "seq2bit")) g->seq2bit = (int)value;
	else if (!strcmp(name, "ring16")) g->ring16 = (int)value;
	else if (!strcmp(name, "band_span") && value >= 0 && value <= 2) g->band_span = (int)value;
	else if (!strcmp(name, "wide_slots") && (value == 0 || value == 3 || value == 4)) g->wide_slots = (int)value;
	else if (!strcmp(name, "lane_max_len")) g->lane_max_len = (int)std::max<int64_t>(0, std::min<int64_t>(value, 8000));
	else if (!strcmp(name, "mid_max_pairs")) g->mid_max_pairs = (int)std::max<int64_t>(-1, std::min<int64_t>(value, 1 << 20));
	else if (!strcmp(name, "host_results")) g->res_pin_on = value != 0;
	else if (!strcmp(name, "div_aware")) g->div_aware = value != 0;
	else if (!strcmp(name, "dev_retry")) g->dev_retry = value != 0;
	else if (!strcmp(name, "band_fold")) g->band_fold = value != 0;
	else if (!strcmp(name, "probe_table")) g->probe_table = value != 0;
	else if (!strcmp(name, "alpha_remap") && (value == 0 || value == 1)) g->alpha_remap = (int)value;
	else if (!strcmp(name, "alpha16") && (value == 0 || value == 1)) g->alpha16 = (int)value;
	else if (!strcmp(name, "trim")) { (void)hipSetDevice(g->device); trim(g); }
	else return -1;
	++g->tun_gen;
	return 0;
}

int mwf_gpu_test_hook(mwf_gpu_t *g, const char *name, int64_t value)
{
	if (!g || !name) return -1;
	if (!strcmp(name, "block")) {
		if (value != 0 && value != 64 && value != 128 && value != 256 && value != 512 && value != 768 && value != 1024) return -1;
		g->block = (int)value;
	} else if (!strcmp(name, "force_kind")) g->force_kind = (int)value;
	else if (!strcmp(name, "band_pack")) g->band_pack = (int)value;
	else if (!strcmp(name, "lane_chunks") && value >= 0 && value <= 4) g->lane_chunks = (int)value;
	else if (!strcmp(name, "mid_block") && (value == 0 || value == 256 || value == 512 || value == 1024)) g->mid_block = (int)value;
	else if (!strcmp(name, "lds_e2")) g->lds_e2 = value != 0;
	else if (!strcmp(name, "probe_table_lds")) g->probe_table_lds = std::max<int64_t>(0, value);
	else if (!strcmp(name, "scalar_generic")) g->scalar_generic = value != 0;
	else if (!strcmp(name, "coop_spin_limit")) g->coop_spin_limit = std::max<int64_t>(0, std::min<int64_t>(value, 0x7fffffff));
	else if (!strcmp(name, "coop_tb_cap_mb")) g->coop_tb_cap = std::max<int64_t>(1, value) << 20;
	else if (!strcmp(name, "coop_grid")) g->coop_grid_cap = (int)std::max<int64_t>(0, value);
	else if (!strcmp(name, "sys_p") && sys_p_supported((int)value)) g->sys_p = (int)value;
	else if (!strcmp(name, "sys_c") && (value == 0 || sys_c_supported((int)value))) g->sys_c = (int)value;
	else if (!strcmp(name, "work_order") && value >= 0 && value <= 3) g->work_order = (int)value;
	else if (!strcmp(name, "alpha_arena_budget")) g->alpha_arena_budget = std::max<int64_t>(-1, value);
	else if (!strcmp(name, "timeline")) g->timeline = (int64_t*)(intptr_t)value;
	else return -1;
	++g->tun_gen;
	return 0;
}

void mwf_gpu_get_stats(const mwf_gpu_t *g, mwf_gpu_stats_t *st)
{
	if (!g || !st) return;
	mwf_gpu_t *m = const_cast<mwf_gpu_t*>(g);
	if (m->ev_pending) {
		(void)hipSetDevice(m->device);
		float ms = 0;
		if (hipEventSynchronize(m->ev1) == hipSuccess && hipEventElapsedTime(&ms, m->ev0, m->ev1) == hipSuccess) m->stats.kernel_ms = ms;
		m->ev_pending = false;
	}
	m->stats.dev_bytes = m->dev_bytes, m->stats.dev_bytes_peak = m->dev_bytes_peak;
	*st = m->stats;
}


mwf_gpu_batch_t *mwf_gpu_batch_upload(mwf_gpu_t *g, int32_t n, const char *seqs, int64_t seq_bytes,
                                      const int64_t *t_off, const int32_t *tl, const int64_t *q_off, const int32_t *ql)
{
	if (!g || n < 0 || seq_bytes < 0) return nullptr;
	return batch_from_host(g, n, tl, nullptr, ql, nullptr, seqs, seq_bytes, t_off, q_off);
}

mwf_gpu_batch_t *mwf_gpu_batch_wrap(mwf_gpu_t *g, int32_t n, const void *d_seqs, int64_t seq_bytes,
                                    const int64_t *d_t_off, const int32_t *d_tl, const int64_t *d_q_off, const int32_t *d_ql,
                                    const int32_t *h_tl, const int32_t *h_ql)
{
	if (!g || n < 0) return nullptr;
	(void)hipSetDevice(g->device);
	BlockLayout L;
	mwf_gpu_batch_t *b = batch_common(g, n, h_tl, h_ql, 0, false, L);
	if (!b) return nullptr;
	b->d_seqs = (const uint8_t*)d_seqs, b->seq_bytes = seq_bytes;
	b->d_t_off = d_t_off, b->d_q_off = d_q_off, b->d_tl = d_tl, b->d_ql = d_ql;
	if (upload_segments(g, (char*)b->block.p, std::vector<Seg>{Seg{b->h_order.data(), (size_t)n * 4}})) {
		mwf_gpu_batch_free(b);
		return nullptr;
	}
	if (g->div_aware) b->div_est = estimate_divergence_device(g, b);
	return b;
}

void mwf_gpu_batch_free(mwf_gpu_batch_t *b)
{
	if (!b) return;
	mwf_gpu_t *g = b->g;
	(void)hipSetDevice(g->device);
	if (b->busy) (void)hipStreamSynchronize(g->stream);
	if (g->res_pin_owner == b) g->res_pin_owner = nullptr;
	give_block(g, g->spare_block, b->block);
	give_block(g, g->spare_cig, b->cig);
	for (DevBuf *d : {&b->ops_summary, &b->ops_map[0], &b->ops_map[1], &b->ops_map_off[0], &b->ops_map_off[1], &b->alpha_cls, &b->alpha_arena, &b->ends_buf}) release(g, *d);
	for (int k = 0; k < MWF_TXT_KINDS; ++k) release(g, b->ops_text[k]), release(g, b->ops_text_off[k]);
	delete b;
}

}


extern "C" {

int mwf_gpu_batch_results(mwf_gpu_t *g, mwf_gpu_batch_t *b, int32_t *s, int64_t *n_iter, int32_t *n_cigar)
{
	if (!g || !b) return -1;
	(void)hipSetDevice(g->device);
	if (int rc = finalize(g, b)) return rc;
	const size_t n = (size_t)b->n;
	if (s && n) memcpy(s, b->h_s.data(), n * 4);
	if (n_iter && n) memcpy(n_iter, b->h_iter.data(), n * 8);
	if (n_cigar && n) memcpy(n_cigar, b->h_ncig.data(), n * 4);
	return 0;
}

const int32_t *mwf_gpu_batch_dev_scores(const mwf_gpu_batch_t *b) { return b ? b->d_s : nullptr; }
const int64_t *mwf_gpu_batch_dev_iters(const mwf_gpu_batch_t *b) { return b ? b->d_iter : nullptr; }
const int32_t *mwf_gpu_batch_dev_status(const mwf_gpu_batch_t *b) { return b ? b->d_status : nullptr; }

const int32_t *mwf_gpu_batch_dev_ranges(const mwf_gpu_batch_t *b) { return b && b->ends_last ? b->d_range : nullptr; }

int mwf_gpu_batch_ranges(mwf_gpu_t *g, mwf_gpu_batch_t *b, int32_t *range)
{
	if (!g || !b || !range) return -1;
	(void)hipSetDevice(g->device);
	if (!b->ends_last) { g->err = "mwf_gpu_batch_ranges: the batch's last align was not ends-free (mwf_gpu_batch_align_ends)"; return -2; }
	if (int rc = finalize(g, b)) return rc;
	if (b->n == 0) return 0;
	return download(g, range, b->d_range, (size_t)b->n * 16);
}

const int32_t *mwf_gpu_batch_dev_ext_info(const mwf_gpu_batch_t *b) { return b && b->ext_last ? b->d_ext_info : nullptr; }

int mwf_gpu_batch_ext_info(mwf_gpu_t *g, mwf_gpu_batch_t *b, int32_t *info)
{
	if (!g || !b || !info) return -1;
	(void)hipSetDevice(g->device);
	if (!b->ext_last) { g->err = "mwf_gpu_batch_ext_info: the batch's last align was not an extension (mwf_gpu_batch_align_ext)"; return -2; }
	if (int rc = finalize(g, b)) return rc;
	if (b->n == 0) return 0;
	return download(g, info, b->d_ext_info, (size_t)b->n * 16);
}

int32_t mwf_gpu_batch_cigar(mwf_gpu_t *g, mwf_gpu_batch_t *b, int32_t i, uint32_t *dst, int32_t cap)
{
	if (!g || !b || i < 0 || i >= b->n) return -1;
	(void)hipSetDevice(g->device);
	if (int rc = finalize(g, b)) return rc;
	const int32_t nc = b->h_ncig[i];
	if (nc > cap) return -5;
	if (nc <= 0) return nc;
	if (b->h_cig_valid) memcpy(dst, b->h_cig.data() + b->h_cigoff[i], (size_t)nc * 4);
	else HIP_TRY(g, hipMemcpy(dst, b->d_cig_pool + b->h_cigoff[i], (size_t)nc * 4, hipMemcpyDeviceToHost));
	return nc;
}

int mwf_gpu_batch_fetch_cigars(mwf_gpu_t *g, mwf_gpu_batch_t *b)
{
	if (!g || !b) return -1;
	(void)hipSetDevice(g->device);
	return fetch_cigars(g, b);
}


static int own_cigars(mwf_gpu_t *g, mwf_gpu_batch_t *b, const char *who)
{
	if (int rc = finalize(g, b)) return rc;
	if (!(b->opt.flag & MWF_F_CIGAR)) { g->err = std::string(who) + ": the batch's last align was score-only (no CIGARs to work on; align with MWF_F_CIGAR)"; return -2; }
	return 0;
}

static int ops_block(mwf_gpu_batch_t *b)
{
	if (b->ops_max_len < 0) {
		b->ops_max_len = 0;
		for (int32_t i = 0; i < b->n; ++i) b->ops_max_len = std::max<int64_t>(b->ops_max_len, (int64_t)b->h_tl[i] + b->h_ql[i]);
	}
	return cigar_ops_block(b->ops_max_len);
}

static CigarOpsArgs ops_args(const mwf_gpu_batch_t *b)
{
	CigarOpsArgs a{};
	a.seqs = b->d_seqs, a.t_off = b->d_t_off, a.q_off = b->d_q_off, a.tl = b->d_tl, a.ql = b->d_ql, a.n_pairs = b->n;
	a.words = b->d_cig_pool, a.word_off = b->d_cigoff, a.n_words = b->d_ncig, a.status = b->d_status;
	if (b->ends_last) a.t_off = b->d_sub_t_off, a.q_off = b->d_sub_q_off, a.tl = b->d_sub_tl, a.ql = b->d_sub_ql;
	return a;
}

int mwf_gpu_batch_dev_cigars(mwf_gpu_t *g, mwf_gpu_batch_t *b, const uint32_t **pool, const int64_t **word_off, const int32_t **n_words, int64_t *pool_words)
{
	if (!g || !b) return -1;
	(void)hipSetDevice(g->device);
	if (int rc = own_cigars(g, b, "mwf_gpu_batch_dev_cigars")) return rc;
	if (pool) *pool = b->d_cig_pool;
	if (word_off) *word_off = b->d_cigoff;
	if (n_words) *n_words = b->d_ncig;
	if (pool_words) *pool_words = b->n > 0 ? b->cig_used : 0;
	return 0;
}

int mwf_gpu_batch_summarize(mwf_gpu_t *g, mwf_gpu_batch_t *b, const mwf_opt_t *opt, const uint32_t *d_words, const int64_t *d_word_off, const int32_t *d_n_words)
{
	if (!g || !b) return -1;
	(void)hipSetDevice(g->device);
	const bool own = !d_words && !d_word_off && !d_n_words;
	if (!own && (!d_words || !d_word_off || !d_n_words)) { g->err = "mwf_gpu_batch_summarize: foreign CIGARs need all three device arrays (words, offsets, counts)"; return -2; }
	if (own) { if (int rc = own_cigars(g, b, "mwf_gpu_batch_summarize")) return rc; }
	else if (b->busy) HIP_TRY(g, hipStreamSynchronize(g->stream));
	if (!opt && !b->aligned) { g->err = "mwf_gpu_batch_summarize: opt == NULL needs an earlier align of the batch"; return -2; }
	const mwf_opt_t &o = opt ? *opt : b->opt;
	b->summary_valid = false;
	if (b->n == 0) { b->summary_valid = true; return 0; }
	if (ensure(g, b->ops_summary, (size_t)b->n * sizeof(mwf_aln_summary_t))) return -1;
	CigarOpsArgs a = ops_args(b);
	if (!own) a.words = d_words, a.word_off = d_word_off, a.n_words = d_n_words, a.status = nullptr, a.t_off = b->d_t_off, a.q_off = b->d_q_off, a.tl = b->d_tl, a.ql = b->d_ql;
	a.x = o.x, a.o1 = o.o1, a.e1 = o.e1, a.o2 = o.o2, a.e2 = o.e2;
	a.mode = 0, a.summary = (int32_t*)b->ops_summary.p;
	if (launch_cigar_ops(a, ops_block(b), g->stream)) { g->err = "kernel launch failed (CIGAR summary)"; return -1; }
	b->summary_valid = true;
	return 0;
}

const mwf_aln_summary_t *mwf_gpu_batch_dev_summary(const mwf_gpu_batch_t *b)
{
	return b && b->summary_valid ? (const mwf_aln_summary_t*)b->ops_summary.p : nullptr;
}

int mwf_gpu_batch_summary(mwf_gpu_t *g, mwf_gpu_batch_t *b, mwf_aln_summary_t *host_out)
{
	if (!g || !b || !host_out) return -1;
	(void)hipSetDevice(g->device);
	if (!b->summary_valid) { g->err = "mwf_gpu_batch_summary: no summary (call mwf_gpu_batch_summarize after the align)"; return -2; }
	return download(g, host_out, b->ops_summary.p, (size_t)b->n * sizeof(mwf_aln_summary_t));
}

int mwf_gpu_batch_map(mwf_gpu_t *g, mwf_gpu_batch_t *b, int32_t which)
{
	if (!g || !b || which < 0 || which > 1) return -1;
	(void)hipSetDevice(g->device);
	if (b->ends_last) { g->err = "mwf_gpu_batch_map: the batch's last align was ends-free (coordinate maps exist for global alignments only)"; return -2; }
	if (int rc = own_cigars(g, b, "mwf_gpu_batch_map")) return rc;
	b->map_valid[which] = false;
	std::vector<int64_t> &off = b->h_map_off[which];
	if (off.empty()) {
		off.assign((size_t)b->n + 1, 0);
		for (int32_t i = 0; i < b->n; ++i) off[i + 1] = off[i] + (which == 0 ? b->h_ql[i] : b->h_tl[i]);
	}
	if (b->n == 0) { b->map_valid[which] = true; return 0; }
	if (ensure(g, b->ops_map[which], std::max<size_t>((size_t)off[b->n] * 4, 256))) return -1;
	if (!b->map_off_uploaded[which]) {
		if (ensure(g, b->ops_map_off[which], ((size_t)b->n + 1) * 8)) return -1;
		if (upload_segments(g, (char*)b->ops_map_off[which].p, std::vector<Seg>{Seg{off.data(), ((size_t)b->n + 1) * 8}})) return -1;
		b->map_off_uploaded[which] = true;
	}
	CigarOpsArgs a = ops_args(b);
	a.mode = 1 + which, a.map = (int32_t*)b->ops_map[which].p, a.map_off = (const int64_t*)b->ops_map_off[which].p;
	if (launch_cigar_ops(a, ops_block(b), g->stream)) { g->err = "kernel launch failed (coordinate map)"; return -1; }
	b->map_valid[which] = true;
	return 0;
}

const int32_t *mwf_gpu_batch_dev_map(const mwf_gpu_batch_t *b, int32_t which)
{
	return b && which >= 0 && which <= 1 && b->map_valid[which] ? (const int32_t*)b->ops_map[which].p : nullptr;
}

int mwf_gpu_batch_map_fetch(mwf_gpu_t *g, mwf_gpu_batch_t *b, int32_t which, int32_t *host_out, int64_t *host_off)
{
	if (!g || !b || which < 0 || which > 1) return -1;
	(void)hipSetDevice(g->device);
	if (!b->map_valid[which]) { g->err = "mwf_gpu_batch_map_fetch: no map (call mwf_gpu_batch_map after the align)"; return -2; }
	const std::vector<int64_t> &off = b->h_map_off[which];
	if (host_off) memcpy(host_off, off.data(), off.size() * 8);
	if (!host_out || b->n == 0) { HIP_TRY(g, hipStreamSynchronize(g->stream)); return 0; }
	return download(g, host_out, b->ops_map[which].p, (size_t)off[b->n] * 4);
}


int mwf_gpu_batch_text(mwf_gpu_t *g, mwf_gpu_batch_t *b, int32_t kind, const uint32_t *d_words, const int64_t *d_word_off, const int32_t *d_n_words)
{
	if (!g || !b) return -1;
	if (kind < 0 || kind >= MWF_TXT_KINDS) { g->err = "mwf_gpu_batch_text: kind must be one of MWF_TXT_* (0 .. 5)"; return -2; }
	(void)hipSetDevice(g->device);
	const bool own = !d_words && !d_word_off && !d_n_words;
	if (!own && (!d_words || !d_word_off || !d_n_words)) { g->err = "mwf_gpu_batch_text: foreign CIGARs need all three device arrays (words, offsets, counts)"; return -2; }
	if (own) { if (int rc = own_cigars(g, b, "mwf_gpu_batch_text")) return rc; }
	else if (b->busy) HIP_TRY(g, hipStreamSynchronize(g->stream));
	b->text_valid[kind] = false;
	DevBuf &off = b->ops_text_off[kind], &pool = b->ops_text[kind];
	if (ensure(g, off, ((size_t)b->n + 1) * 8)) return -1;
	CigarTextArgs a{};
	a.seqs = b->d_seqs, a.t_off = b->d_t_off, a.q_off = b->d_q_off, a.tl = b->d_tl, a.ql = b->d_ql, a.n_pairs = b->n;
	a.words = b->d_cig_pool, a.word_off = b->d_cigoff, a.n_words = b->d_ncig, a.status = b->d_status;
	if (!own) a.words = d_words, a.word_off = d_word_off, a.n_words = d_n_words, a.status = nullptr;
	else if (b->ends_last) a.t_off = b->d_sub_t_off, a.q_off = b->d_sub_q_off, a.tl = b->d_sub_tl, a.ql = b->d_sub_ql;
	a.kind = kind, a.off = (int64_t*)off.p;
	const int block = ops_block(b);
	a.mode = 0;
	if (launch_cigar_text(a, block, g->stream) || launch_text_scan(a.off, b->n, g->stream)) { g->err = "kernel launch failed (alignment text, sizing)"; return -1; }
	int64_t total = 0;
	if (int rc = download(g, &total, a.off + b->n, 8)) return rc;
	if (total < 0) { g->err = "mwf_gpu_batch_text: negative text size"; return -1; }
	if (ensure(g, pool, std::max<size_t>((size_t)total, 256))) return -1;
	a.mode = 1, a.txt = (char*)pool.p;
	if (launch_cigar_text(a, block, g->stream)) { g->err = "kernel launch failed (alignment text)"; return -1; }
	b->text_total[kind] = total;
	b->text_valid[kind] = true;
	return 0;
}

const char *mwf_gpu_batch_dev_text(const mwf_gpu_batch_t *b, int32_t kind, const int64_t **d_off, int64_t *total)
// ... 363 lines not shown
```

### miniwfa_amd/csrc/mwf_engine.h

```cpp
#pragma once
#include <hip/hip_runtime.h>
#include <algorithm>
#include <cstdio>
#include <cstdlib>
#include <cstring>
#include <map>
#include <mutex>
#include <shared_mutex>
#include <numeric>
#include <string>
#include <chrono>
#include <cmath>
#include <functional>
#include <thread>
#include <tuple>
#include <vector>
#include "miniwfa.h"
#include "kalloc.h"
#include "mwf_internal.h"
#include "mwf_ends.h"
#include "mwf_plan_classes.h"

namespace mwf {
namespace host {


[[noreturn]] inline void fatal(const char *what, const char *detail)
{
	fprintf(stderr, "[libmwf_hip] fatal: %s%s%s\n", what, detail ? ": " : "", detail ? detail : "");
	abort();
}

struct DevBuf {
	void *p = nullptr;
	size_t bytes = 0;
};

constexpr size_t kPinHalfMax = (size_t)16 << 20;
constexpr int kCigBlock = 256, kCigBlockGrid = 8192, kCigBlockPairs = 4096;
constexpr int kQueueSlots = 64;
constexpr int kLaneCounters = 64, kLaneStride = 32, kLaneSets = 4, kQueueInts = kQueueSlots + kLaneSets * kLaneCounters * kLaneStride;
constexpr int kMaxDevices = 64;

inline size_t align_up(size_t v, size_t a) { return (v + a - 1) / a * a; }

struct OccKey {
	int kind = 0, block = 0;
	bool ext = false;
	int packed = 0, lane = 0, slots512 = 0, e1 = 0, e2 = 0, lds_bytes = 0;
	bool cigar = false, seq2 = false, tab = false, nib = false;
	bool stream_pass = false, ring16 = false, big_ring = false;
	int lds_e2_cols = 0;
	auto tied() const { return std::tie(kind, block, ext, packed, lane, slots512, e1, e2, lds_bytes, cigar, seq2, tab, nib, stream_pass, ring16, big_ring, lds_e2_cols); }
	bool operator<(const OccKey &o) const { return tied() < o.tied(); }
};


}
}

using namespace mwf;
using namespace mwf::host;


struct mwf_gpu_s {
	int device = 0;
	hipStream_t stream = nullptr;
	bool own_stream = false;
	int n_cu = 0;
	size_t total_mem = 0;
	std::string err;
	int block = 0;
	bool dev_retry = true;
	bool band_fold = true;
	bool probe_table = true;
	int64_t probe_table_lds = 0;
	bool div_aware = true;
	int64_t tun_gen = 0;
	int64_t coop_min_len = 0;
	int64_t tb_budget_mb = 0;
	int force_kind = -1;
	int work_order = 1;
	int64_t *timeline = nullptr;
	int res_pin_on = 1;
	int lane_chunks = 0;
	int lane_max_len = 325;
	int mid_max_pairs = -1;
	int mid_block = 0;
	int band_pack = -1;
	int wide_slots = 0;
	int band_span = 1;
	int ring16 = 1;
	int seq2bit = 1;
	int alpha_remap = 0;
	int alpha16 = 0;
	int64_t alpha_arena_budget = -1;
	int lds_e2 = 1;
	int scalar_generic = 0;
	int64_t coop_spin_limit = 1 << 23;
	int64_t coop_tb_cap = (int64_t)96 << 30;
	int64_t coop_tb_mult = 1;
	int64_t lowmem_budget_mb = 0;
	int sys_p = 8;
	int sys_c = 0;
	DevBuf ring, sring, good, tb, row_off, row_lo, cig_scratch, snap, snap_meta, seg, queue, dbg, coop_misc;
	DevBuf retry_ids;
	DevBuf sys_box, sys_prog, sys_log, sys_ep, sys_park, sys_ring, sys_sring, sys_good;
	DevBuf spare_block, spare_cig;
	int queue_next = 0;
	int lane_set_next = 0;
	bool queue_clean = false;
	void *pin = nullptr;
	size_t pin_half = 0;
	hipEvent_t pin_ev[2] = {nullptr, nullptr};
	void *res_pin = nullptr;
	const void *res_pin_owner = nullptr;
	bool pin_busy[2] = {false, false};
	hipEvent_t ev0 = nullptr, ev1 = nullptr;
	bool ev_pending = false;
	hipEvent_t ev_alpha[4] = {nullptr, nullptr, nullptr, nullptr};
	bool alpha_timed[2] = {false, false};
	mwf_gpu_stats_t stats{};
	int64_t dev_bytes = 0, dev_bytes_peak = 0;
	std::map<OccKey, int> occ_cache;
	int coop_grid = -1;
	int coop_grid_cap = 0;
};

struct mwf_gpu_batch_s {
	mwf_gpu_t *g = nullptr;
	int32_t n = 0;
	bool owns_inputs = false;
	DevBuf block;
	const uint8_t *d_seqs = nullptr;
	int64_t seq_bytes = 0;
	const int64_t *d_t_off = nullptr, *d_q_off = nullptr;
	const int32_t *d_tl = nullptr, *d_ql = nullptr;
	std::vector<int32_t> h_tl, h_ql;
	int64_t max_seq_lds = 0;
	int64_t max_tl = 0;
	int32_t *d_order = nullptr;
	std::vector<int32_t> h_order;
	std::vector<int32_t> h_len_order;
	std::vector<int8_t> h_class;
	std::vector<int8_t> h_kind;
	float div_est = 0;
	std::vector<int8_t> h_acgt;
	std::vector<int8_t> h_acgt_host;
	std::vector<int8_t> h_alpha;
	std::vector<uint32_t> h_sym;
	std::vector<int8_t> h_alpha_up;
	int alpha16_laid_out = -1;
	DevBuf alpha_cls;
	DevBuf alpha_arena;
	const int64_t *d_rt_off = nullptr, *d_rq_off = nullptr;
	bool alpha_known = false;
	bool alpha_active = false;
	bool alpha_laid_out = false;
	std::vector<int8_t> h_flags;
	unsigned long long *d_cig_head = nullptr;
	int32_t *d_status = nullptr, *d_s = nullptr, *d_ncig = nullptr, *d_dbg4 = nullptr;
	int64_t *d_iter = nullptr, *d_cigoff = nullptr, *d_cells1 = nullptr;
	size_t out_off = 0, out_bytes = 0;
	bool out_in_pin = false;
	bool results_preinit = false;
	DevBuf cig;
	uint32_t *d_cig_pool = nullptr;
	int64_t cig_pool_words = 0;
	int32_t cig_block = 0;
	bool aligned = false, finalized = false, busy = false;
	mwf_opt_t opt{};
	std::vector<int32_t> h_s, h_ncig, h_status;
	std::vector<int64_t> h_iter, h_cigoff, h_cells1;
	int64_t cig_used = 0;
	int32_t cig_block_left = 0;
	std::vector<uint32_t> h_cig;
	bool h_cig_valid = false;
	struct PlanCache {
		bool valid = false;
		int32_t opt_key[8] = {0, 0, 0, 0, 0, 0, 0, 0};
		int64_t tun_key[3] = {0, 0, 0};
		int64_t max_len = 0, max_bound = 0;
		bool has_groups = false, mid_bytes = false;
		int8_t wide_state = 0;
		bool wide_measured = false;
		struct GI {
			int32_t n = 0;
			int64_t max_len = 0, max_bound = 0, max_bound1 = 0, max_tl = 0, max_seq_lds = 0, max_exp_win = 0;
			void add(int64_t tl, int64_t ql, const int64_t &bound, const int64_t &bound1, const int64_t &exp_win)
			{
				++n;
				max_len = std::max(max_len, tl + ql), max_bound = std::max(max_bound, bound), max_bound1 = std::max(max_bound1, bound1);
				max_tl = std::max(max_tl, tl), max_exp_win = std::max(max_exp_win, exp_win);
				max_seq_lds = std::max<int64_t>(max_seq_lds, ((tl + 3) & ~3LL) + 8 + ((ql + 3) & ~3LL) + 16);
			}
		} gi[kNumClasses];
		std::vector<int8_t> cls0, flags0;
	} plan;
	std::vector<char> host_out;
	size_t out_bytes_score = 0;
	int32_t last_grid = 0, n_retries = 0;
	int32_t *d_retry_ids = nullptr;
	bool dev_retry_used = false;
	int32_t debug_pair = -1;
	DevBuf ops_summary, ops_map[2], ops_map_off[2];
	bool summary_valid = false, map_valid[2] = {false, false};
	std::vector<int64_t> h_map_off[2];
	bool map_off_uploaded[2] = {false, false};
	DevBuf ops_text[MWF_TXT_KINDS], ops_text_off[MWF_TXT_KINDS];
	bool text_valid[MWF_TXT_KINDS] = {false, false, false, false, false, false};
	int64_t text_total[MWF_TXT_KINDS] = {0, 0, 0, 0, 0, 0};
	int64_t ops_max_len = -1;
	bool ends_last = false;
	bool ext_last = false;
	mwf_ends_t ends{};
	mwf_ext_t ext{};
	DevBuf ends_buf;
	int32_t *d_range = nullptr, *d_ext_info = nullptr, *d_sub_tl = nullptr, *d_sub_ql = nullptr, *d_ends_order = nullptr;
	int64_t *d_sub_t_off = nullptr, *d_sub_q_off = nullptr;
};


#define HIP_TRY(g, call)                                                              \
	do {                                                                              \
		hipError_t e_ = (call);                                                       \
		if (e_ != hipSuccess) {                                                       \
			(g)->err = std::string(#call) + ": " + hipGetErrorString(e_);             \
			return -1;                                                                \
		}                                                                             \
	} while (0)

namespace mwf {
namespace host {

void account(mwf_gpu_t *g, int64_t delta);
int ensure(mwf_gpu_t *g, DevBuf &b, size_t bytes);
void release(mwf_gpu_t *g, DevBuf &b);
int take_block(mwf_gpu_t *g, DevBuf &spare, DevBuf &out, size_t bytes);
void give_block(mwf_gpu_t *g, DevBuf &spare, DevBuf &b);
int pin_reserve(mwf_gpu_t *g, size_t half);
struct Seg { const void *src; size_t len; };
int upload_segments(mwf_gpu_t *g, char *dst, const std::vector<Seg> &segs);
int download(mwf_gpu_t *g, void *dst, const void *src, size_t bytes);
struct BlockLayout {
	size_t order = 0, t_off = 0, q_off = 0, tl = 0, ql = 0, seqs = 0, in_end = 0;
	size_t head = 0, status = 0, s = 0, ncig = 0, iter = 0, cigoff = 0, cells1 = 0, score_end = 0, out_end = 0, dbg4 = 0, retry = 0, total = 0;
};
constexpr int kRetryCap = 256;
constexpr int kRetrySlots = 2;
BlockLayout layout_block(size_t n, size_t seq_bytes, bool owned);
mwf_gpu_batch_t *batch_common(mwf_gpu_t *g, int32_t n, const int32_t *h_tl, const int32_t *h_ql, size_t seq_bytes, bool owned, BlockLayout &L);
mwf_gpu_batch_t *batch_from_host(mwf_gpu_t *g, int32_t n, const int32_t *tl, const char *const *ts, const int32_t *ql, const char *const *qs,
                                 const char *packed, int64_t packed_bytes, const int64_t *p_t_off, const int64_t *p_q_off);
float estimate_divergence_device(mwf_gpu_t *g, mwf_gpu_batch_t *b);
int alpha_prepare(mwf_gpu_t *g, mwf_gpu_batch_t *b);
int alphabet_scan16(const uint8_t *t, size_t tl, const uint8_t *q, size_t ql, uint8_t sym[16]);
int alphabet_scan(const uint8_t *t, size_t tl, const uint8_t *q, size_t ql, uint8_t sym[4]);
double sketch_divergence(int32_t hit, int32_t tot, int32_t lt);
extern "C" int mwf_gpu_test_hook(mwf_gpu_t *g, const char *name, int64_t value);
int64_t coalesce_window_us();
void exact_coalesced(void *km, const mwf_opt_t *opt, int32_t tl, const char *ts, int32_t ql, const char *qs, mwf_rst_t *r);

Penalty make_penalty(const mwf_opt_t &o);
const char *validate(const mwf_opt_t &o);
int64_t penalty_bound(const mwf_opt_t &o, int64_t tl, int64_t ql, bool honour_max_s);
int coop_grid_limit(mwf_gpu_t *g);
int finalize(mwf_gpu_t *g, mwf_gpu_batch_t *b);
int fetch_cigars(mwf_gpu_t *g, mwf_gpu_batch_t *b);

}
}
```

### miniwfa_amd/csrc/mwf_internal.h

```cpp
#pragma once
#include <stdint.h>

namespace mwf {

constexpr int32_t kNegInf = -0x40000000;
constexpr int32_t kMaxRing = 256;
constexpr int32_t kBigRing = 4096;

enum : int32_t {
	ST_OK = 0,
	ST_STOPPED = 1,
	ST_TB_OVERFLOW = 2,
	ST_ROWS_OVERFLOW = 3,
	ST_CIGAR_OVERFLOW = 4,
	ST_SNAP_OVERFLOW = 5,
	ST_INTERNAL = 6,
	ST_PENDING = 7,
	ST_BAND_OVERFLOW = 8,
	ST_ALPHABET = 9
};

struct Penalty {
	int32_t x;
	int32_t oe1;
	int32_t e1;
	int32_t oe2;
	int32_t e2;
	int32_t o1, o2;
	int32_t nH;
	int32_t n1;
	int32_t n2;
};

struct BatchArgs {
	const uint8_t *seqs;
	const int64_t *t_off, *q_off;
	const int32_t *tl, *ql;
	const int32_t *order;
	int32_t n_pairs;
	int32_t *queue;
	int32_t queue_parts;
	Penalty pen;
	int32_t want_cigar;
	int32_t step;
	int32_t max_s;
	int64_t max_iter;
	int32_t debug_pair;
	int32_t *ring;
	int32_t *sring;
	int64_t ring_slot_ints;
	int32_t W;
	unsigned long long *good;
	int32_t GW;
	uint8_t *tb;
	int64_t tb_slot_bytes;
	int64_t *row_off;
	int32_t *row_lo;
	int64_t rows_slot;
	uint32_t *cig_scratch;
	int64_t cig_scratch_slot;
	uint32_t *cig_pool;
	unsigned long long *cig_head;
	int64_t cig_pool_words;
	int32_t *snap;
	int64_t snap_slot_ints;
	int32_t *snap_meta;
	int64_t snap_meta_slot;
	int32_t *seg;
	int64_t seg_slot;
	int32_t *out_s;
	int64_t *out_iter;
	int32_t *out_ncig;
	int64_t *out_cigoff;
	int32_t *out_status;
	int64_t *out_cells1;
	int32_t *out_dbg;
	int32_t *dbg;
	int32_t dbg_cap;
	int32_t coop_pair;
	int32_t lds_e2_cols;
	int32_t ring16;
	int32_t scalar_generic;
	int32_t band_lds_seq;
	int32_t band_fold;
	int32_t coop_groups, coop_group_size;
	int64_t coop_edge_stride;
	int64_t coop_sedge_off;
	int64_t coop_misc_stride;
	const int32_t *coop_pair_ids;
	uint32_t coop_spin_limit;
	int32_t *retry_ids;
	unsigned int *retry_count;
	int32_t retry_cap;
	const unsigned int *n_pairs_dev;
	int32_t coop_pass;
	int32_t *coop_edge;
	int32_t *coop_flags;
	unsigned int *coop_sync;
	int32_t *coop_state;
	int32_t sys_p;
	int32_t sys_c;
	int32_t sys_spread;
	int32_t *sys_box;
	int64_t sys_box_stride;
	unsigned long long *sys_prog;
	int64_t sys_prog_stride;
	int32_t *sys_log;
	int64_t sys_log_stride;
	int32_t *sys_park;
	int64_t sys_park_stride;
	int64_t *sys_ep;
	int64_t sys_ep_stride;
	int32_t report_wide;
	int32_t cig_block;
	int32_t lane_chunks;
	int32_t sys_coop_launch;
	int64_t *timeline;
	int32_t band_lds_tab;
};

int launch_batch(const BatchArgs &a, int grid, int block, void *stream);
int launch_reset(int32_t *status, int32_t *s, int32_t n, unsigned long long *cig_head, int32_t *queue, int32_t n_queue, void *stream);
int launch_sketch(const uint8_t *seqs, const int64_t *t_off, const int32_t *tl, const int64_t *q_off, const int32_t *ql, int32_t n, int32_t samples, int32_t *out, void *stream);
int launch_pair_sketch(const uint8_t *seqs, const int64_t *t_off, const int32_t *tl, const int64_t *q_off, const int32_t *ql, const int32_t *order, int32_t n, int32_t *out, void *stream);
struct CigarOpsArgs {
	const uint8_t *seqs;
	const int64_t *t_off, *q_off;
	const int32_t *tl, *ql;
	int32_t n_pairs;
	const uint32_t *words;
	const int64_t *word_off;
	const int32_t *n_words;
	const int32_t *status;
	int32_t x, o1, e1, o2, e2;
	int32_t mode;
	int32_t *summary;
	int32_t *map;
	const int64_t *map_off;
};
int cigar_ops_block(int64_t max_len);
int launch_cigar_ops(const CigarOpsArgs &a, int block, void *stream);
struct CigarTextArgs {
	const uint8_t *seqs;
	const int64_t *t_off, *q_off;
	const int32_t *tl, *ql;
	int32_t n_pairs;
	const uint32_t *words;
	const int64_t *word_off;
	const int32_t *n_words;
	const int32_t *status;
	int32_t kind;
	int32_t mode;
	int64_t *off;
	char *txt;
};
int launch_cigar_text(const CigarTextArgs &a, int block, void *stream);
int launch_text_scan(int64_t *off, int32_t n, void *stream);
struct AlphabetArgs {
	const uint8_t *seqs;
	const int64_t *t_off, *q_off;
	const int32_t *tl, *ql;
	const int32_t *ids;
	int32_t n_pairs;
	int32_t mode;
	int32_t alpha16;
	int8_t *cls;
	uint32_t *sym;
	const int64_t *dst_t, *dst_q;
	int64_t *out_t_off, *out_q_off;
};
constexpr int kAlphaSymWords = 4;
int alphabet_block(int64_t max_len);
int launch_alphabet(const AlphabetArgs &a, int block, void *stream);
int  bigring_kernel_occupancy();
int  batch_kernel_occupancy(int block, bool stream_pass, int lds_e2_cols, bool ring16);

struct BandGeom {
	int block;
	int packed;
	int span;
	int lds_bytes;
	int seq2;
	int lane;
	int tab;
	int nib;
};
bool coop_supported(const Penalty &p);
int64_t coop_chunk_slots(int grid);
int64_t sys_chunk_slots(int grid);
int  sys_owned_cols(int p, int c);
bool sys_c_supported(int c);
bool sys_p_supported(int p);
constexpr int64_t sys_box_ints(int p, int nef, bool seg) { return ((seg ? 4 : 2) * p * (p + nef) + 2 * p + 31) / 32 * 32; }
constexpr int64_t sys_park_ints(int nef, bool seg) { return (int64_t)(seg ? 2 : 1) * nef * 64 * 4; }
constexpr int kSysNotResident = -3;
int  sys_max_grid();
int  launch_sys_pass(const BatchArgs &a, int grid, void *stream);
int  launch_sys_pass_deep(const BatchArgs &a, int grid, void *stream);
int  launch_sys_walk(const BatchArgs &a, void *stream);
int  launch_sys_trace(const BatchArgs &a, void *stream);
int  launch_sys_finish(const BatchArgs &a, void *stream);

bool lane_supported(const Penalty &p);
int  lane_lds_bytes(const Penalty &p, int chunks, int64_t seq_bytes);
int  launch_lane(const BatchArgs &a, int grid, int lds, bool seq2, void *stream);
int  lane_kernel_occupancy(int lds, bool cigar);

bool mid_supported(const Penalty &p);
int  mid_lds_bytes(const Penalty &p, int groups, int64_t seq_bytes);
int  launch_mid(const BatchArgs &a, int grid, int block, int lds, bool seq2, void *stream);

bool band2_supported(const Penalty &p);
int  launch_band2(const BatchArgs &a, int grid, const BandGeom &g, void *stream);
int  band2_kernel_occupancy(const Penalty &p, const BandGeom &g, bool cigar);
int  launch_band2_e3(const BatchArgs &a, int grid, const BandGeom &g, void *stream);
int  launch_band2_e4(const BatchArgs &a, int grid, const BandGeom &g, void *stream);
int  launch_band2_bi1(const BatchArgs &a, int grid, const BandGeom &g, void *stream);
int  launch_band2_bi2(const BatchArgs &a, int grid, const BandGeom &g, void *stream);
int  launch_band2_tab(const BatchArgs &a, int grid, const BandGeom &g, void *stream);
int  launch_band2_nib(const BatchArgs &a, int grid, const BandGeom &g, void *stream);
int  band2_occupancy_e3(const Penalty &p, const BandGeom &g, bool cigar);
int  band2_occupancy_e4(const Penalty &p, const BandGeom &g, bool cigar);
int  band2_occupancy_bi1(const Penalty &p, const BandGeom &g, bool cigar);
int  band2_occupancy_bi2(const Penalty &p, const BandGeom &g, bool cigar);
int  band2_occupancy_tab(const Penalty &p, const BandGeom &g, bool cigar);
int  band2_occupancy_nib(const Penalty &p, const BandGeom &g, bool cigar);
bool band2_nib_supported(const Penalty &p);
bool band2_tab_supported(const Penalty &p, bool band_fold);
bool band2_biased512_supported(const Penalty &p);
int  band2_biased512_chunks();
int  band2_span_chunks();

}
```

### miniwfa_amd/csrc/mwf_plan.cpp

```cpp
#include "mwf_engine.h"
#include "mwf_plan_retry.h"

namespace mwf {
namespace host {


Penalty make_penalty(const mwf_opt_t &o)
{
	Penalty p;
	p.x = o.x, p.o1 = o.o1, p.o2 = o.o2, p.e1 = o.e1, p.e2 = o.e2;
	p.oe1 = o.o1 + o.e1, p.oe2 = o.o2 + o.e2;
	int32_t mp = std::max(p.x, std::max(p.oe1, p.oe2));
	p.nH = mp + 1, p.n1 = p.e1 + 1, p.n2 = p.e2 + 1;
	return p;
}

const char *validate(const mwf_opt_t &o)
{
	if (o.x < 1 || o.e1 < 1 || o.e2 < 1) return "x, e1 and e2 must be >= 1 (a zero lag would make a wavefront depend on itself)";
	if (o.o1 < 0 || o.o2 < 0) return "gap-open penalties must be >= 0";
	if (std::max<int64_t>(o.x, std::max<int64_t>((int64_t)o.o1 + o.e1, (int64_t)o.o2 + o.e2)) + 1 > kBigRing) return "max(x, o1+e1, o2+e2) must be < 4096";
	if (o.step < 0) return "step must be >= 0";
	return nullptr;
}

int64_t penalty_bound(const mwf_opt_t &o, int64_t tl, int64_t ql, bool honour_max_s) { return penalty_bound(make_penalty(o), o.max_s, tl, ql, honour_max_s); }

inline int64_t band_span_window() { return band_window(band2_span_chunks()); }

struct SlotSizes {
	int32_t W = 0, GW = 0;
	int64_t ring_slot_ints = 0, rows_slot = 0, cig_scratch_slot = 0, tb_slot_bytes = 0;
};

struct Plan {
	int kind = 0;
	BandGeom band{0, 0, 0, 0, 0, 0};
	int block = 256, grid = 1;
	SlotSizes ws;
	int64_t snap_slot_ints = 0, snap_meta_slot = 0, seg_slot = 0;
	bool low_mem = false, cigar = false;
	bool ext = false;
};

typedef mwf_gpu_batch_t::PlanCache::GI GroupInfo;

static auto longer_first(const mwf_gpu_batch_t *b)
{
	return [b](int32_t x, int32_t y) { return (int64_t)b->h_tl[x] + b->h_ql[x] > (int64_t)b->h_tl[y] + b->h_ql[y]; };
}

struct LaunchReq {
	mwf_opt_t opt{};
	const int32_t *d_order = nullptr;
	int32_t n_items = 0;
	int slots = 1 << 30;
	GroupInfo group;
	Geom geom = GEOM_CHOOSE;
	CopyForm copy = COPY_2BIT;
	int want_kind = -1;
	int64_t window_hint = 0;
	bool ring16_allowed = true;
	int retry_list = 0;
	int retry_slot = 0;
	bool report_wide = false;
	bool timed_begin = false, timed_end = false;
};

int cached_occupancy(mwf_gpu_t *g, const Penalty &P, const Plan &pl, int lds_e2_cols, bool stream_pass, bool ring16 = false);

void choose_kernel(mwf_gpu_t *g, const LaunchReq &rq, const Penalty &P, Plan &pl)
{
	const mwf_opt_t &opt = rq.opt;
	const int want_kind = rq.want_kind >= 0 ? rq.want_kind : g->force_kind;
	const int64_t max_len = rq.group.max_len, max_bound = rq.group.max_bound, max_seq_lds = rq.group.max_seq_lds, max_tl = rq.group.max_tl, window_hint = rq.window_hint;
	Geom geom = rq.geom;
	const bool bytes_only = rq.copy == COPY_BYTES;
	pl.kind = 0;
	const bool low_mem = (opt.flag & MWF_F_CIGAR) && opt.step > 0;
	const bool can_packed = band2_supported(P) && g->band_pack != 0;
	if (geom == GEOM_LANE && want_kind != 0 && !low_mem && lane_supported(P)) {
		const int chunks = g->lane_chunks > 0 ? g->lane_chunks : max_len <= 400 ? 3 : 4;
		BandGeom lg{64, 1, 64 * chunks, lane_lds_bytes(P, chunks, max_seq_lds), (g->seq2bit != 0 && !bytes_only && max_len >= 450) ? 1 : 0, 1};
		if (lg.lds_bytes <= 60 * 1024) {
			pl.kind = 2, pl.band = lg;
			return;
		}
	}
	if (geom == GEOM_MID && want_kind != 0 && !low_mem && mid_supported(P)) {
		const int64_t want_cols = (std::min<int64_t>(max_len + 1, 2 * max_bound + 3) + 2 * P.nH + 63) / 64 * 64;
		int groups = (int)std::min<int64_t>(want_cols / 64, 128);
		while (groups > 1 && mid_lds_bytes(P, groups, max_seq_lds) > 158 * 1024) --groups;
		const int lds = mid_lds_bytes(P, groups, max_seq_lds);
		if (lds <= 158 * 1024) {
			const int64_t by_len = window_hint > 0 ? std::max<int64_t>(max_len, window_hint * 100 / 28) : max_len;
			const int block = g->mid_block ? g->mid_block : (by_len <= 1000 ? 256 : by_len <= 2500 ? 512 : 1024);
			const int seq2 = g->seq2bit != 0 && !bytes_only;
			pl.kind = 2, pl.band = BandGeom{block, 1, 64 * groups, lds, seq2, 2};
			return;
		}
	}
	if (want_kind == 0 || low_mem || !can_packed) return;
	if (geom == GEOM_BIASED) {
		const int64_t need_lds = ((max_len >> 4) + 4) * 4;
		if (g->seq2bit == 0 || bytes_only || need_lds > 70 * 1024 || !band2_biased512_supported(P)) return;
		const bool six = max_len + 1 > 7 * (int64_t)(band2_biased512_chunks() * 256) / 2 || (window_hint > 0 && window_hint + 768 > ((int64_t)band2_biased512_chunks() - 1) * 256 - 64);
		const int chunks = band2_biased512_chunks() + (six ? 8 : 0);
		pl.kind = 2, pl.band = BandGeom{512, 2, chunks * 256, (int)((need_lds + 15) / 16 * 16), 1, 0};
		pl.cigar = (opt.flag & MWF_F_CIGAR) != 0;
		if (cached_occupancy(g, P, pl, 0, false) >= 2) return;
		pl.kind = 0, pl.band = BandGeom{0, 0, 0, 0, 0, 0}, geom = GEOM_SPAN;
	}
	if (geom == GEOM_SPAN) {
		const bool nib = rq.copy == COPY_NIB && band2_nib_supported(P);
		const int64_t need_lds = nib ? ((max_len >> 3) + 4) * 4 : ((max_len >> 4) + 4) * 4;
		if (g->band_span == 0 || g->seq2bit == 0 || bytes_only || need_lds > 150 * 1024) return;
		pl.kind = 2, pl.band = BandGeom{1024, 1, (int)band2_span_chunks() * 256, (int)((need_lds + 15) / 16 * 16), 1, 0, 0, nib ? 1 : 0};
		return;
	}
	const int64_t max_window = window_hint > 0 ? std::min<int64_t>(std::min<int64_t>(max_len + 1, 2 * max_bound + 3), window_hint) : std::min<int64_t>(max_len + 1, 2 * max_bound + 3);
	BandGeom bg;
	bg.packed = 0, bg.seq2 = 0, bg.lane = 0, bg.tab = 0, bg.nib = 0;
	const bool range_ok = max_tl + max_bound < 32767;
	if (!range_ok) return;
	bg.packed = 1;
	bg.block = max_window <= kBandMicroWindow ? 64 : max_window <= kBandTinyWindow ? 128 : max_window <= kBandSmallWindow ? 256 : 512;
	if (g->block == 64 || g->block == 128 || g->block == 256 || g->block == 512 || g->block == 768) bg.block = g->block;
	if (g->block == 0 && geom_small_block(geom)) bg.block = geom_small_block(geom);
	const bool nib = rq.copy == COPY_NIB && g->seq2bit != 0 && !bytes_only && band2_nib_supported(P) && bg.block != 768;
	if (nib) bg.block = 512;
	bg.span = bg.block / 64 * (bg.block != 768 ? 3 : 2) * 256;
	const bool four_slots = bg.block == 512 && ((g->block == 0 && window_hint > kBandWideWindow && window_hint <= kBandWide4Window) || (g->block == 512 && g->wide_slots == 4));
	if (four_slots) bg.span = 512 / 64 * 4 * 256;
	if (want_kind != 2 && max_len + 1 > 4 * (int64_t)bg.span) return;
	const int64_t lds_cap = bg.block >= 768 ? 140 * 1024 : bg.block >= 512 ? 70 * 1024 : bg.block == 256 ? 36 * 1024 : bg.block == 128 ? 18 * 1024 : 9 * 1024;
	const bool seq2 = g->seq2bit != 0 && !bytes_only;
	const int64_t need_lds = nib ? ((max_len >> 3) + 4) * 4 : seq2 ? ((max_len >> 4) + 4) * 4 : max_seq_lds;
	bg.lds_bytes = need_lds <= lds_cap ? (int)((need_lds + 15) / 16 * 16) : 0;
	bg.seq2 = seq2 && bg.lds_bytes > 0;
	if (bg.block == 768) bg.seq2 = 0, bg.lds_bytes = max_seq_lds <= 140 * 1024 ? (int)((max_seq_lds + 15) / 16 * 16) : 0;
	else if (!bg.seq2) {
		bg.block = 768, bg.span = 768 / 64 * 2 * 256;
		bg.lds_bytes = max_seq_lds <= 140 * 1024 ? (int)((max_seq_lds + 15) / 16 * 16) : 0;
	}
	if (bg.lds_bytes == 0) return;
	bg.nib = nib && bg.seq2 && bg.block == 512;
	pl.kind = 2, pl.band = bg;
	if (g->probe_table && bg.block == 512 && bg.seq2 && !bg.nib && band2_tab_supported(P, g->band_fold)) {
		const int64_t tab = (2 * (max_len + 258) + 15) / 16 * 16;
		const int64_t budget = g->probe_table_lds > 0 ? g->probe_table_lds : (160 / 2 - 6) * 1024;
		if (tab + bg.lds_bytes <= budget) {
			pl.band.tab = (int)tab, pl.band.lds_bytes = (int)(tab + bg.lds_bytes);
			pl.cigar = (opt.flag & MWF_F_CIGAR) != 0;
			if (cached_occupancy(g, P, pl, 0, false) < 2) pl.band = bg;
		}
	}
}

int cached_occupancy(mwf_gpu_t *g, const Penalty &P, const Plan &pl, int lds_e2_cols, bool stream_pass, bool ring16)
{
	OccKey key;
	if (pl.kind == 3) key.kind = 3, key.block = pl.block, key.ext = pl.ext;
	else if (pl.kind == 2) {
		key.kind = 2, key.block = pl.band.block, key.packed = pl.band.packed, key.lane = pl.band.lane, key.slots512 = pl.band.block == 512 ? pl.band.span / 2048 : 0;
		key.e1 = P.e1, key.e2 = P.e2, key.lds_bytes = pl.band.lds_bytes, key.cigar = pl.cigar, key.seq2 = pl.band.seq2 != 0, key.tab = pl.band.tab > 0, key.nib = pl.band.nib != 0;
	} else key.block = pl.block, key.stream_pass = stream_pass, key.ring16 = ring16, key.big_ring = P.nH > kMaxRing, key.lds_e2_cols = lds_e2_cols;
	auto it = g->occ_cache.find(key);
	if (it != g->occ_cache.end()) return it->second;
	const int per = pl.kind == 3 ? ends_kernel_occupancy(pl.block, pl.ext)
	              : pl.kind == 2 && pl.band.lane == 2 ? 1
	              : pl.kind == 2 && pl.band.lane ? lane_kernel_occupancy(pl.band.lds_bytes, pl.cigar)
	              : pl.kind == 2 ? band2_kernel_occupancy(P, pl.band, pl.cigar)
	              : P.nH > kMaxRing ? bigring_kernel_occupancy()
	                             : batch_kernel_occupancy(pl.block, stream_pass, lds_e2_cols, ring16);
	g->occ_cache[key] = per;
	return per;
}

int64_t tb_budget_bytes(mwf_gpu_t *g)
{
	if (g->tb_budget_mb > 0) return g->tb_budget_mb << 20;
	size_t fr = 0, tot = 0;
	if (hipMemGetInfo(&fr, &tot) != hipSuccess) fr = (size_t)8 << 30, tot = fr;
	int64_t b = (int64_t)(fr / 5 * 4) + (int64_t)g->tb.bytes;
	return std::min<int64_t>(b, std::min<int64_t>((int64_t)64 << 30, (int64_t)(tot / 4)));
}

std::shared_mutex g_dev_gate[kMaxDevices];


static int window_block(const GroupInfo &G) { return std::min<int64_t>(G.max_len + 1, 2 * G.max_bound + 3) >= 8192 ? 512 : 256; }
static void set_row_stride(SlotSizes &ws, int64_t max_len) { ws.W = (int32_t)((max_len + 3 + 255) / 256 * 256 + 512), ws.GW = ws.W / 64 + 2; }
static int64_t tb_worst(const GroupInfo &G) { return (G.max_bound + 1) * (G.max_len + 1) + 8 * (G.max_bound + 2); }

static int size_slots(mwf_gpu_t *g, const Penalty &P, const GroupInfo &G, int grid, bool cigar, int64_t worst, bool rings_in_lds, SlotSizes &ws)
{
	set_row_stride(ws, G.max_len);
	ws.ring_slot_ints = rings_in_lds ? 64 : (int64_t)(P.nH + 2 * P.n1 + 2 * P.n2) * ws.W;
	const size_t S = (size_t)grid;
	if (ensure(g, g->ring, S * ws.ring_slot_ints * 4)) return -1;
	if (ensure(g, g->good, S * (size_t)P.nH * ws.GW * 8)) return -1;
	if (!cigar) return 0;
	ws.rows_slot = G.max_bound + 2, ws.cig_scratch_slot = G.max_len + 2;
	int64_t per = worst;
	if ((int64_t)g->tb.bytes < (int64_t)S * worst || g->tb_budget_mb > 0) per = std::min(per, std::max<int64_t>(tb_budget_bytes(g), (int64_t)g->tb.bytes) / (int64_t)S);
	if (g->tb_budget_mb > 0) per = std::min(per, (g->tb_budget_mb << 20) / (int64_t)S);
	ws.tb_slot_bytes = std::max<int64_t>(4096, per) / 4 * 4;
	if (ensure(g, g->tb, S * (size_t)ws.tb_slot_bytes)) return -1;
	if (ensure(g, g->row_off, S * (size_t)ws.rows_slot * 8)) return -1;
	if (ensure(g, g->row_lo, S * (size_t)ws.rows_slot * 4)) return -1;
	return ensure(g, g->cig_scratch, S * (size_t)ws.cig_scratch_slot * 4);
}

static void fill_args(BatchArgs &a, const mwf_gpu_t *g, const mwf_gpu_batch_t *b, const mwf_opt_t &opt, const Penalty &P, bool cigar, const SlotSizes &ws, bool remapped)
{
	a.seqs = b->d_seqs, a.t_off = remapped ? b->d_rt_off : b->d_t_off, a.q_off = remapped ? b->d_rq_off : b->d_q_off, a.tl = b->d_tl, a.ql = b->d_ql;
	a.pen = P, a.want_cigar = cigar ? 1 : 0, a.max_s = opt.max_s, a.max_iter = opt.max_iter;
	a.debug_pair = b->debug_pair;
	a.ring = (int32_t*)g->ring.p, a.ring_slot_ints = ws.ring_slot_ints, a.W = ws.W, a.good = (unsigned long long*)g->good.p, a.GW = ws.GW;
	a.tb = cigar ? (uint8_t*)g->tb.p : nullptr, a.tb_slot_bytes = ws.tb_slot_bytes;
	a.row_off = cigar ? (int64_t*)g->row_off.p : nullptr, a.row_lo = cigar ? (int32_t*)g->row_lo.p : nullptr, a.rows_slot = ws.rows_slot;
	a.cig_scratch = cigar ? (uint32_t*)g->cig_scratch.p : nullptr, a.cig_scratch_slot = ws.cig_scratch_slot;
	a.cig_pool = b->d_cig_pool, a.cig_head = b->d_cig_head, a.cig_pool_words = b->cig_pool_words;
	a.out_s = b->d_s, a.out_iter = b->d_iter, a.out_ncig = b->d_ncig, a.out_cigoff = b->d_cigoff;
	a.out_status = b->d_status, a.out_cells1 = b->d_cells1, a.out_dbg = b->d_dbg4;
}

static int take_counter(mwf_gpu_t *g, int32_t *&queue)
{
	if (g->queue_clean && g->queue_next < kQueueSlots) { queue = (int32_t*)g->queue.p + g->queue_next++; return 0; }
	queue = (int32_t*)g->queue.p;
	HIP_TRY(g, hipMemsetAsync(g->queue.p, 0, 4, g->stream));
	return 0;
}

template <class Launch>
static int launch_gated(mwf_gpu_t *g, mwf_gpu_batch_t *b, const LaunchReq &rq, const Plan &pl, int packed, const char *what, Launch launch)
{
	if (rq.timed_begin) HIP_TRY(g, hipEventRecord(g->ev0, g->stream));
	std::shared_lock<std::shared_mutex> gate(g_dev_gate[g->device % kMaxDevices]);
	const int lrc = launch();
	gate.unlock();
	if (lrc != 0) { g->err = what; return -1; }
	b->last_grid = std::max(b->last_grid, pl.grid);
	if (rq.timed_end) HIP_TRY(g, hipEventRecord(g->ev1, g->stream));
	g->ev_pending |= rq.timed_end;
	g->stats.n_launches += 1;
	g->stats.grid = std::max(g->stats.grid, pl.grid), g->stats.block = pl.block, g->stats.kernel_kind = pl.kind;
	g->stats.packed = packed, g->stats.lowmem_two_pass = pl.low_mem ? 1 : 0;
	return 0;
}

int run_batch_kernel(mwf_gpu_t *g, mwf_gpu_batch_t *b, const LaunchReq &rq, int *ran_kind)
{
	const mwf_opt_t &opt = rq.opt;
	const int32_t n_items = rq.n_items;
	const int64_t max_len = rq.group.max_len, max_bound = rq.group.max_bound, max_bound1 = rq.group.max_bound1, max_tl = rq.group.max_tl;
	int slots = rq.slots;
	const Penalty P = make_penalty(opt);
	Plan pl;
	pl.cigar = (opt.flag & MWF_F_CIGAR) != 0;
	pl.low_mem = pl.cigar && opt.step > 0;
	pl.block = g->block > 0 && g->block != 768 ? g->block : window_block(rq.group);
	choose_kernel(g, rq, P, pl);
	int per_cu, lds_e2_cols = 0;
	bool ring16 = false;
	if (pl.kind == 2) {
		pl.block = pl.band.block;
		per_cu = cached_occupancy(g, P, pl, 0, false);
	} else {
		if (g->lds_e2 && pl.block == 512 && g->block == 0 && P.e2 == 1 && !g->scalar_generic && !pl.low_mem && P.nH <= kMaxRing) {
			lds_e2_cols = 16384;
			const int64_t s_guess = b->div_est > 0 && g->div_aware ? (int64_t)(6.9 * b->div_est * (double)max_tl) + 256 : max_len / 8;
			ring16 = g->ring16 != 0 && rq.ring16_allowed && max_tl + std::max<int64_t>(s_guess, max_len / 8) < 65500;
			pl.block = ring16 ? (pl.cigar ? 768 : 512) : 768;
		}
		if (P.nH > kMaxRing) pl.block = 256;
		per_cu = cached_occupancy(g, P, pl, lds_e2_cols, !g->scalar_generic, ring16);
	}
	slots = std::max(1, std::min(slots, g->n_cu * std::max(1, per_cu)));
	if (P.nH > kMaxRing) {
		const int64_t per_slot = (int64_t)(P.nH + 2 * P.n1 + 2 * P.n2) * ((max_len + 3 + 255) / 256 * 256 + 512) * 4 * (pl.low_mem ? 2 : 1);
		slots = (int)std::max<int64_t>(1, std::min<int64_t>(slots, (int64_t)(g->total_mem / 10) / std::max<int64_t>(per_slot, 1)));
	}
	pl.grid = std::max(1, std::min<int>(slots, n_items));
	if (getenv("MWF_DEBUG"))
		fprintf(stderr, "[libmwf_hip] kernel kind %d: block %d packed %d lds %d B, %d workgroup(s) per CU, %d slots, %d pairs; span %d seq2 %d lane %d tab %d nib %d grid %d hint %lld\n", pl.kind, pl.block,
		        pl.band.packed, pl.band.lds_bytes, per_cu, slots, n_items, pl.band.span, pl.band.seq2, pl.band.lane, pl.band.tab, pl.band.nib, pl.grid, (long long)rq.window_hint);
	int64_t worst = tb_worst(rq.group);
	if (pl.low_mem && opt.step > 2 * P.nH) worst = std::min(worst, (max_bound + 1) * std::min<int64_t>(max_len + 1, 2 * (int64_t)(opt.step + 2 * P.nH) + 8) + 8 * (max_bound + 2));
	if (pl.kind == 2 && pl.band.lane == 1) worst = (std::min<int64_t>(max_bound, 256) + 2) * pl.band.span;
	if (pl.kind == 2 && pl.band.lane == 2) worst = (max_bound + 2) * pl.band.span;
	if (size_slots(g, P, rq.group, pl.grid, pl.cigar, worst, pl.kind == 2 && pl.band.lane, pl.ws)) return -1;
	const size_t S = (size_t)pl.grid;
	if (pl.low_mem) {
		const int64_t NS = P.nH + 2 * P.n1 + 2 * P.n2;
		const int64_t n_snap_max = max_bound1 / opt.step + 2;
		pl.seg_slot = n_snap_max;
		pl.snap_meta_slot = n_snap_max * (4 + 4 * NS);
		int64_t worst = 0;
		for (int64_t j = 1; j <= n_snap_max; ++j)
			worst += NS * std::min<int64_t>(max_len + 1, 2 * j * opt.step + 3);
		const int64_t budget = (int64_t)(std::max<int64_t>(tb_budget_bytes(g), (int64_t)g->snap.bytes) / 4 / (int64_t)S);
		pl.snap_slot_ints = std::max<int64_t>(1024, std::min(worst, budget));
		if (ensure(g, g->sring, S * pl.ws.ring_slot_ints * 4)) return -1;
		if (ensure(g, g->snap, S * (size_t)pl.snap_slot_ints * 4)) return -1;
		if (ensure(g, g->snap_meta, S * (size_t)pl.snap_meta_slot * 4)) return -1;
		if (ensure(g, g->seg, S * (size_t)pl.seg_slot * 8)) return -1;
	}

	BatchArgs a;
	memset(&a, 0, sizeof(a));
	fill_args(a, g, b, opt, P, pl.cigar, pl.ws, b->alpha_active);
	a.order = rq.d_order, a.n_pairs = n_items;
	a.timeline = g->timeline;
	if (pl.kind == 2 && pl.band.lane == 1 && n_items > pl.grid) {
		a.queue_parts = kLaneCounters;
		if (g->queue_clean && g->lane_set_next < kLaneSets) a.queue = (int32_t*)g->queue.p + kQueueSlots + (g->lane_set_next++) * kLaneCounters * kLaneStride;
		else {
			a.queue = (int32_t*)g->queue.p + kQueueSlots;
			HIP_TRY(g, hipMemsetAsync(a.queue, 0, (size_t)kLaneCounters * kLaneStride * 4, g->stream));
		}
	} else if (pl.kind == 2 && pl.band.lane == 1) a.queue = nullptr;
	else if (pl.kind == 2 && (pl.band.lane || pl.band.packed) && n_items <= pl.grid && !g->queue_clean) a.queue = nullptr;
	else if (take_counter(g, a.queue)) return -1;
	if (rq.retry_list == 1) a.retry_ids = b->d_retry_ids + rq.retry_slot * kRetryCap, a.retry_cap = kRetryCap, a.retry_count = (unsigned int*)(b->d_cig_head + 2 + rq.retry_slot);
	if (rq.retry_list == 2) a.n_pairs_dev = (const unsigned int*)(b->d_cig_head + 2 + rq.retry_slot), a.queue = nullptr, a.queue_parts = 0;
	a.scalar_generic = g->scalar_generic;
	a.band_fold = g->band_fold ? 1 : 0;
	a.lds_e2_cols = lds_e2_cols;
	a.ring16 = ring16 ? 1 : 0;
	a.lane_chunks = pl.kind == 2 && pl.band.lane ? pl.band.span / 64 : 0;
	a.step = pl.low_mem ? opt.step : 0;
	a.sring = pl.low_mem ? (int32_t*)g->sring.p : nullptr;
	a.cig_block = 0;
	if (b->cig_block > 0 && pl.grid <= b->cig_block_left) a.cig_block = b->cig_block, b->cig_block_left -= pl.grid;
	a.report_wide = rq.report_wide ? 1 : 0;
	a.snap = pl.low_mem ? (int32_t*)g->snap.p : nullptr, a.snap_slot_ints = pl.snap_slot_ints;
	a.snap_meta = pl.low_mem ? (int32_t*)g->snap_meta.p : nullptr, a.snap_meta_slot = pl.snap_meta_slot;
	a.seg = pl.low_mem ? (int32_t*)g->seg.p : nullptr, a.seg_slot = pl.seg_slot;
	a.dbg = b->debug_pair >= 0 ? (int32_t*)g->dbg.p : nullptr;
	a.dbg_cap = b->debug_pair >= 0 ? (int32_t)(g->dbg.bytes / 8) : 0;

	const int packed = pl.kind == 2 ? (pl.band.lane == 2 ? 33 : pl.band.lane ? 32 : (pl.band.packed ? 1 : 0)) : (ring16 ? 16 : 0);
	if (ran_kind) *ran_kind = pl.kind;
	return launch_gated(g, b, rq, pl, packed, "kernel launch failed", [&] {
		return pl.kind == 2 && pl.band.lane == 2 ? launch_mid(a, pl.grid, pl.band.block, pl.band.lds_bytes, pl.band.seq2 != 0, g->stream)
		     : pl.kind == 2 && pl.band.lane ? launch_lane(a, pl.grid, pl.band.lds_bytes, pl.band.seq2 != 0, g->stream)
		     : pl.kind == 2 ? launch_band2(a, pl.grid, pl.band, g->stream)
		                    : launch_batch(a, pl.grid, pl.block, g->stream);
	});
}

int run_ends_kernel(mwf_gpu_t *g, mwf_gpu_batch_t *b, const LaunchReq &rq, int *ran_kind)
{
	const mwf_opt_t &opt = rq.opt;
	const Penalty P = make_penalty(opt);
	Plan pl;
	pl.kind = 3, pl.cigar = (opt.flag & MWF_F_CIGAR) != 0, pl.block = window_block(rq.group);
	pl.ext = b->ext_last;
	const int per_cu = cached_occupancy(g, P, pl, 0, false);
	const int slots = std::max(1, std::min(rq.slots, g->n_cu * std::max(1, per_cu)));
	pl.grid = std::max(1, std::min<int>(slots, rq.n_items));
	if (size_slots(g, P, rq.group, pl.grid, pl.cigar, tb_worst(rq.group), false, pl.ws)) return -1;
	if (getenv("MWF_DEBUG"))
		fprintf(stderr, "[libmwf_hip] kernel kind 3: block %d, %d workgroup(s) per CU, %d slots, %d pairs; grid %d, traceback %lld B per slot\n", pl.block, per_cu, slots, rq.n_items, pl.grid, (long long)pl.ws.tb_slot_bytes);

	EndsArgs e;
	memset(&e, 0, sizeof(e));
	BatchArgs &a = e.b;
	fill_args(a, g, b, opt, P, pl.cigar, pl.ws, false);
	a.order = rq.d_order, a.n_pairs = rq.n_items;
	if (take_counter(g, a.queue)) return -1;
	a.debug_pair = -1, a.out_dbg = nullptr;
	e.t_beg = b->ends.t_beg, e.t_end = b->ends.t_end, e.q_beg = b->ends.q_beg, e.q_end = b->ends.q_end;
	e.out_range = b->d_range, e.sub_t_off = b->d_sub_t_off, e.sub_q_off = b->d_sub_q_off, e.sub_tl = b->d_sub_tl, e.sub_ql = b->d_sub_ql;
	e.ext = pl.ext, e.match = b->ext.match, e.zdrop = b->ext.zdrop, e.out_info = b->d_ext_info;
	if (ran_kind) *ran_kind = 3;
	return launch_gated(g, b, rq, pl, 0, "kernel launch failed (ends-free)", [&] { return launch_ends(e, pl.grid, pl.block, g->stream); });
}



int coop_grid_limit(mwf_gpu_t *g)
{
	if (g->coop_grid < 0) g->coop_grid = std::min(sys_max_grid(), g->n_cu);
	return g->coop_grid_cap > 0 ? std::min(g->coop_grid, g->coop_grid_cap) : g->coop_grid;
}

int coop_group_size(int n_cu, int64_t len, bool alone, int ow = 256)
{
	int G = n_cu;
	const int64_t chunks = alone ? len / ow + (ow == 256 ? 3 : 8) : len / ow / 3 + (ow == 256 ? 8 : 12);
	while (G > (alone ? 64 : 16) && chunks <= coop_chunk_slots(G / 2)) G /= 2;
	return G;
}

int run_coop_group(mwf_gpu_t *g, mwf_gpu_batch_t *b, const mwf_opt_t &opt, const std::vector<int32_t> &pairs, int Gs, bool first, bool last)
{
	const Penalty P = make_penalty(opt);
	const bool cigar = (opt.flag & MWF_F_CIGAR) != 0, low_mem = cigar && opt.step > 0;
	const int n_groups = (int)pairs.size();
	if (n_groups < 1 || Gs < 1 || (int64_t)Gs * n_groups > coop_grid_limit(g)) { g->err = "whole-device kernel cannot be made resident"; return -1; }
	GroupInfo M;
	bool traced = false;
	for (int32_t pair : pairs) {
		M.add(b->h_tl[pair], b->h_ql[pair], penalty_bound(opt, b->h_tl[pair], b->h_ql[pair], true), penalty_bound(opt, b->h_tl[pair], b->h_ql[pair], false), 0);
		traced |= b->debug_pair == pair;
	}
	const int64_t len = M.max_len, bound = M.max_bound, bound1 = M.max_bound1;
	SlotSizes ws;
	set_row_stride(ws, len);
	ws.ring_slot_ints = (int64_t)P.nH * ws.W;
	const int64_t TC = coop_chunk_slots(Gs);
	const size_t NG = (size_t)n_groups;
	const int sysP = g->sys_p, sysP2 = g->sys_p;
	auto window_cap = [&](int c) -> int64_t { return (TC - 4) * (int64_t)sys_owned_cols(sysP, c) - 2 * (257 + sysP); };
	bool wide_again = false;
	for (int32_t pair : pairs) wide_again |= (b->h_flags[pair] & FLAG_COOP_WIDE) != 0;
	const int64_t est1 = std::min<int64_t>(len + 1, std::max<int64_t>(8192, b->div_est > 0 && g->div_aware ? (int64_t)(6.5 * b->div_est * (double)len) : len / 5));
	const int64_t est2 = std::min<int64_t>(len + 1, 2 * ((int64_t)opt.step + 2 * P.nH) + 8);
	const int c_first = g->sys_c ? g->sys_c : (!wide_again && est1 <= window_cap(1)) ? 1 : 4;
	const int c_second = g->sys_c ? g->sys_c : (!wide_again && est2 <= window_cap(1)) ? 1 : 4;
	bool two_pass = false;
	if (low_mem) {
		const int64_t budget = g->lowmem_budget_mb > 0 ? g->lowmem_budget_mb << 20 : (int64_t)8 << 30;
		two_pass = std::max<int64_t>((int64_t)1 << 30, 6000 * len) * (int64_t)NG * g->coop_tb_mult * (c_first == 1 ? 12 : 9) / 8 > budget;
	}
	const size_t misc_bytes = 4096;
	if (ensure(g, g->coop_misc, NG * misc_bytes + 4096)) return -1;
	int64_t rows_slot = 0, tb_bytes = 0, cig_scratch = 0, seg_slot = 0;
	if (cigar) {
		rows_slot = std::max(bound, bound1) + 2;
		cig_scratch = len + 2;
		const int64_t worst = NG * (rows_slot + 1) * (len + 8);
		int64_t guess = std::min<int64_t>(g->coop_tb_cap, std::max<int64_t>((int64_t)1 << 30, 6000 * len) * (int64_t)NG);
		if (two_pass) guess = std::min<int64_t>(guess, std::max<int64_t>((int64_t)64 << 20, (len * 3 / 100 + 1024) * std::min<int64_t>(len + 1, 2 * (int64_t)(opt.step + 2 * P.nH) + 8)) * (int64_t)NG);
		const int64_t lay = (two_pass ? c_second : c_first) == 1 ? 12 : (two_pass ? c_second : c_first) == 2 ? 10 : 9;
		const int64_t ep_guess = (len * 3 / 100 + 1024) / 256 + 2;
		guess = std::min<int64_t>(g->coop_tb_cap, guess / 8 * lay + ep_guess * 8 * 65536 * (int64_t)NG);
		int64_t want = std::min(worst / 8 * lay + (rows_slot / 256 + 2) * 8 * 65536 * (int64_t)NG, g->tb_budget_mb > 0 ? (g->tb_budget_mb << 20) : guess * g->coop_tb_mult);
		if ((int64_t)g->tb.bytes >= want) want = (int64_t)g->tb.bytes;
		else {
			size_t fr = 0, tot = 0;
			if (hipMemGetInfo(&fr, &tot) != hipSuccess) fr = (size_t)8 << 30;
			want = std::min<int64_t>(want, (int64_t)(fr / 10 * 9) + (int64_t)g->tb.bytes);
		}
		tb_bytes = std::max<int64_t>(4096, want / (int64_t)NG) / 4 * 4;
		if (ensure(g, g->row_off, NG * (size_t)rows_slot * 8)) return -1;
		if (ensure(g, g->row_lo, NG * (size_t)rows_slot * 4)) return -1;
		if (ensure(g, g->cig_scratch, NG * (size_t)cig_scratch * 4)) return -1;
		if (low_mem) {
			seg_slot = bound1 / opt.step + 2;
			if (ensure(g, g->seg, NG * (size_t)seg_slot * 8)) return -1;
		}
		if (ensure(g, g->tb, NG * (size_t)tb_bytes)) return -1;
	}
	int64_t snap_slot_ints = 0, snap_meta_slot = 0;
	if (two_pass) {
		const int64_t NS = P.nH + 2 * P.e1 + 2 * P.e2, s_guess = len * 3 / 100 + 1024, n_guess = s_guess / opt.step + 2;
		int64_t cols = 0;
		for (int64_t j = 1; j <= n_guess; ++j) cols += std::min<int64_t>(len + 1, 2 * j * opt.step) + 1100;
		snap_meta_slot = (bound1 / opt.step + 256 / opt.step + 4) * 8;
		snap_slot_ints = std::min<int64_t>(std::max<int64_t>((int64_t)4 << 20, NS * cols) * g->coop_tb_mult, ((int64_t)48 << 30) / 4) / 4 * 4;
		if (ensure(g, g->sys_sring, NG * (size_t)TC * P.nH * 256 * 4)) return -1;
		if (ensure(g, g->snap, NG * (size_t)snap_slot_ints * 4)) return -1;
		if (ensure(g, g->snap_meta, NG * (size_t)snap_meta_slot * 4)) return -1;
	}
// ... 710 lines not shown
```

Before: 1.805 Gbp/s.

## Add second-fold table kernel folding the O2 open row into E2/F2

Adds a new band2 kernel form (tab2) for score-only e2==1 penalties. It stops loading the O2 neighbour row and N2, and folds the O2 contribution into the E2/F2 gap values one penalty ahead by reading the ring at a lag shortened by e2. The E2/F2 edge exchange is split into half-writes placed after the extension step. The aim is fewer LDS/ring loads and fewer max operations per cell. In exchange the kernel ages cells out later, adds a second edge-write phase, and is a separate specialised kernel only chosen when occupancy allows.

After: 1.886 Gbp/s (median of 6 runs). 4.5% higher.

```diff
diff --git a/miniwfa_amd/build.py b/miniwfa_amd/build.py
--- a/miniwfa_amd/build.py
+++ b/miniwfa_amd/build.py
@@ -8,9 +8,10 @@
 ROOT = os.path.dirname(HERE)
 CSRC = os.path.join(HERE, "csrc")
 LIB = os.path.join(CSRC, "libmwf_hip.so")
-SOURCES = ["mwf_band2.hip", "mwf_band2_tab.hip", "mwf_band2_nib.hip", "mwf_band2_e3.hip", "mwf_band2_e4.hip", "mwf_band2_bi.hip", "mwf_band2_bi_deep.hip", "mwf_kernels.hip", "mwf_sketch.hip", "mwf_ends.hip", "mwf_lane.hip", "mwf_mid.hip", "mwf_sys.hip", "mwf_sys_deep.hip", "mwf_cigar_ops.hip", "mwf_cigar_text.hip", "mwf_alphabet.hip", "mwf_engine.cpp", "mwf_memory.cpp", "mwf_plan.cpp", "mwf_chain.cpp", "mwf_async.cpp", "kalloc.cpp", "mwf_dbg.cpp"]
+SOURCES = ["mwf_band2.hip", "mwf_band2_tab.hip", "mwf_band2_nib.hip", "mwf_band2_e3.hip", "mwf_band2_e4.hip", "mwf_band2_bi.hip", "mwf_band2_bi_deep.hip", "mwf_band2_tab2.hip", "mwf_kernels.hip", "mwf_sketch.hip", "mwf_ends.hip", "mwf_lane.hip", "mwf_mid.hip", "mwf_sys.hip", "mwf_sys_deep.hip", "mwf_cigar_ops.hip", "mwf_cigar_text.hip", "mwf_alphabet.hip", "mwf_engine.cpp", "mwf_memory.cpp", "mwf_plan.cpp", "mwf_chain.cpp", "mwf_async.cpp", "kalloc.cpp", "mwf_dbg.cpp"]
 HEADERS = [os.path.join(CSRC, "mwf_internal.h"), os.path.join(CSRC, "mwf_device.h"), os.path.join(CSRC, "mwf_ends.h"), os.path.join(CSRC, "mwf_sys_pass.h"), os.path.join(CSRC, "mwf_band2_kernel.h"), os.path.join(CSRC, "mwf_band2_dispatch.h"), os.path.join(CSRC, "mwf_engine.h"), os.path.join(CSRC, "mwf_plan_classes.h"), os.path.join(CSRC, "mwf_plan_retry.h"), os.path.join(ROOT, "include", "miniwfa.h"), os.path.join(ROOT, "include", "kalloc.h")]
-BAND2_UNITS = [s for s in SOURCES if s.startswith("mwf_band2")]
+BAND2_FOLD2_UNITS = ["mwf_band2_tab2.hip"]
+BAND2_UNITS = [s for s in SOURCES if s.startswith("mwf_band2") and s not in BAND2_FOLD2_UNITS]
 
 
 def hipcc() -> str:
@@ -66,9 +67,9 @@
     return LIB
 
 
-KERNEL_FILES = {"wfa_band2_kernel": "mwf_band2_kernel.h", "wfa_band2_tab_kernel": "mwf_band2_kernel.h", "wfa_band2_nib_kernel": "mwf_band2_kernel.h", "wfa_sys_kernel": "mwf_sys.hip", "wfa_sys_seg_kernel": "mwf_sys.hip",
+KERNEL_FILES = {"wfa_band2_kernel": "mwf_band2_kernel.h", "wfa_band2_tab_kernel": "mwf_band2_kernel.h", "wfa_band2_nib_kernel": "mwf_band2_kernel.h", "wfa_band2_tab2_kernel": "mwf_band2_kernel.h", "wfa_sys_kernel": "mwf_sys.hip", "wfa_sys_seg_kernel": "mwf_sys.hip",
                 "wfa_batch_kernel": "mwf_kernels.hip", "wfa_lane_kernel": "mwf_lane.hip", "wfa_mid_kernel": "mwf_mid.hip", "wfa_ends_kernel": "mwf_ends.hip"}
-KERNEL_HEADERS = {"mwf_sys.hip": ["mwf_sys_pass.h", "mwf_sys_deep.hip"], "mwf_band2_kernel.h": ["mwf_band2_dispatch.h", *BAND2_UNITS]}
+KERNEL_HEADERS = {"mwf_sys.hip": ["mwf_sys_pass.h", "mwf_sys_deep.hip"], "mwf_band2_kernel.h": ["mwf_band2_dispatch.h", *BAND2_UNITS, *BAND2_FOLD2_UNITS]}
 
 
 def kernel_fingerprint(symbol: str) -> str | None:
@@ -105,7 +106,7 @@
 
 if __name__ == "__main__":
     if "--list-band-units" in sys.argv or "--list-sources" in sys.argv:
-        print(" ".join(BAND2_UNITS if "--list-band-units" in sys.argv else SOURCES))
+        print(" ".join(BAND2_UNITS + BAND2_FOLD2_UNITS if "--list-band-units" in sys.argv else SOURCES))
         sys.exit(0)
     print(build(force="--force" in sys.argv, verbose=True))
     print(build_cli(force="--force" in sys.argv))
diff --git a/miniwfa_amd/csrc/mwf_band2.hip b/miniwfa_amd/csrc/mwf_band2.hip
--- a/miniwfa_amd/csrc/mwf_band2.hip
+++ b/miniwfa_amd/csrc/mwf_band2.hip
@@ -35,6 +35,10 @@
 	BandGeom g = g0;
 	if (g.nib) return launch_band2_nib(a, grid, g, stream);
 	if (g.tab > 0) {
+		if (g.fold2) {
+			const int rc2 = launch_band2_tab2(a, grid, g, stream);
+			if (rc2 != -1) return rc2;
+		}
 		const int rc = launch_band2_tab(a, grid, g, stream);
 		if (rc != -1) return rc;
 		g.lds_bytes -= g.tab, g.tab = 0;
@@ -48,6 +52,7 @@
 int band2_kernel_occupancy(const Penalty &p, const BandGeom &g, bool cigar)
 {
 	if (g.nib) return band2_occupancy_nib(p, g, cigar);
+	if (g.tab > 0 && g.fold2 && !cigar) return band2_occupancy_tab2(p, g, cigar);
 	if (g.tab > 0) return band2_occupancy_tab(p, g, cigar);
 	if (g.packed == 2 && !has_pen_set(MainBiasedSets{}, p.e1, p.e2)) return p.e1 <= 2 ? band2_occupancy_bi1(p, g, cigar) : band2_occupancy_bi2(p, g, cigar);
 	if (p.e1 == 3) return band2_occupancy_e3(p, g, cigar);
diff --git a/miniwfa_amd/csrc/mwf_band2_dispatch.h b/miniwfa_amd/csrc/mwf_band2_dispatch.h
--- a/miniwfa_amd/csrc/mwf_band2_dispatch.h
+++ b/miniwfa_amd/csrc/mwf_band2_dispatch.h
@@ -32,6 +32,7 @@
 using BiDeepSets = PenSets<PenSet<3, 1>, PenSet<3, 2>, PenSet<4, 1>>;
 using TabSets = PenSets<PenSet<2, 1>>;
 using NibSets = PenSets<PenSet<2, 1>>;
+using Tab2Sets = PenSets<PenSet<2, 1>>;
 using NoSets = PenSets<>;
 
 template <int T_, int K_, bool BI4_ = false> struct Geo { static constexpr int T = T_, K = K_; static constexpr bool BI4 = BI4_; };
diff --git a/miniwfa_amd/csrc/mwf_band2_kernel.h b/miniwfa_amd/csrc/mwf_band2_kernel.h
--- a/miniwfa_amd/csrc/mwf_band2_kernel.h
+++ b/miniwfa_amd/csrc/mwf_band2_kernel.h
@@ -12,6 +12,8 @@
 #define MWF_BAND2_KERNEL wfa_band2_tab_kernel
 #elif MWF_BAND2_FORM == 2
 #define MWF_BAND2_KERNEL wfa_band2_nib_kernel
+#elif MWF_BAND2_FORM == 3
+#define MWF_BAND2_KERNEL wfa_band2_tab2_kernel
 #else
 #define MWF_BAND2_KERNEL wfa_band2_kernel
 #endif
@@ -34,7 +36,9 @@
 constexpr int kChunk = 256;
 constexpr int kFoldMaxLag = 8;
 constexpr int32_t kDeadPair = (int32_t)0x80008000u;
-constexpr bool kTabProbe = MWF_BAND2_FORM == 1;
+constexpr bool kTabProbe = MWF_BAND2_FORM == 1 || MWF_BAND2_FORM == 3;
+constexpr bool kFold2Form = MWF_BAND2_FORM == 3;
+constexpr int kFold2MaxLag = 16;
 constexpr bool kNib = MWF_BAND2_FORM == 2;
 constexpr int kSeqSh = kNib ? 2 : 1, kSeqDw = kNib ? 3 : 4, kSeqPer = 1 << kSeqDw;
 constexpr uint32_t kNibTag = 0x40;
@@ -270,8 +274,11 @@
 	constexpr int FULL = TAB ? 8 : S2 ? kSeqPer : 8;
 	constexpr bool kChain = TAB;
 	constexpr bool kGeo = TAB && band2_geo_cached(T, K, TB);
+	constexpr bool kFold2 = kFold2Form && TAB && FOLD && !TB && E2 == 1;
+	static_assert(!kFold2Form || kFold2, "the second fold exists on the table form, folded, score-only, e2 == 1");
 #define MWF_RARE(x) (kChain ? __builtin_expect((x), 0) != 0 : (x))
-	constexpr int kAgeOut = FOLD ? kFoldMaxLag : D;
+	constexpr int kAgeOut = kFold2 ? kFold2MaxLag - E2 + D : FOLD ? kFoldMaxLag : D;
+	static_assert(!kFold2 || (kAgeOut >= kFoldMaxLag && kAgeOut < 128), "the second fold ages at least as long as the first; two shrinks are 256 penalties apart");
 	constexpr int kAge = (NWK + 2) * 16;
 	static_assert(D >= 2 && D <= 5, "edge-table ages");
 	const int32_t tl = M.tl, ql = M.ql, cmax = tl + ql + 1;
@@ -281,7 +288,8 @@
 	const int32_t ONEB = BI ? both16(1 + B) : 0x00010001;
 	char *const Hb = (char*)M.H;
 	const uint32_t RS = (uint32_t)W << 1;
-	const int32_t min_lag = min(lagx, min(lag1, lag2));
+	const int32_t lag2r = kFold2 ? lag2 - E2 : lag2;
+	const int32_t min_lag = min(lagx, min(lag1, lag2r));
 	const bool relaxed_stores = min_lag >= 3;
 	PassResult R;
 	R.status = ST_OK, R.s = 0, R.info = 0, R.n_snap = 0, R.cells = 0;
@@ -339,13 +347,13 @@
 	int32_t s = 0, wf_lo = tl + 1, wf_hi = tl + 1;
 	int32_t curH = 0, par = 0;
 	const uint32_t ring_bytes = (uint32_t)nH * RS;
-	uint32_t bn = (uint32_t)(1 % nH) * RS, bx = (uint32_t)((nH - lagx + 1) % nH) * RS, b1 = (uint32_t)((nH - lag1 + 1) % nH) * RS, b2 = (uint32_t)((nH - lag2 + 1) % nH) * RS;
+	uint32_t bn = (uint32_t)(1 % nH) * RS, bx = (uint32_t)((nH - lagx + 1) % nH) * RS, b1 = (uint32_t)((nH - lag1 + 1) % nH) * RS, b2 = (uint32_t)((nH - lag2r + 1) % nH) * RS;
 	struct Rows { int2 HX, O1, O2; int32_t N1, N2; } pre;
 	pre.HX = pre.O1 = pre.O2 = make_int2(0, 0), pre.N1 = pre.N2 = 0;
 	auto load_rows = [&](Rows &r, const char *rx, const char *r1, const char *r2, uint32_t off) {
 		const uint32_t noff = off + (uint32_t)nd;
 		r.HX = *(const int2*)(rx + off), r.O2 = *(const int2*)(r2 + off);
-		r.N2 = *(const int32_t*)(r2 + noff);
+		if (!kFold2) r.N2 = *(const int32_t*)(r2 + noff);
 		if (!FOLD) r.O1 = *(const int2*)(r1 + off), r.N1 = *(const int32_t*)(r1 + noff);
 	};
 	const int64_t iter_limit = A.max_iter > 0 ? A.max_iter : INT64_MAX;
@@ -468,6 +476,12 @@
 			*(int2*)(lds2 + wF + (k * NW + 1) * 16 + 8) = make_int2(f1a, f2a);
 			if (k == K - 1 && wave == NW - 1) *(int2*)(lds2 + wE - (NW - 1) * 16) = make_int2(e1b, e2b);
 			if (k == 0 && wave == 0) *(int2*)(lds2 + wF + (NWK + 1) * 16 + 8) = make_int2(f1a, f2a);
+		};
+		auto put_edge_half = [&](int k, int h, int32_t eb, int32_t fa) {
+			*(int32_t*)(lds2 + wE + (k * NW + 1) * 16 + 4 * h) = eb;
+			*(int32_t*)(lds2 + wF + (k * NW + 1) * 16 + 8 + 4 * h) = fa;
+			if (k == K - 1 && wave == NW - 1) *(int32_t*)(lds2 + wE - (NW - 1) * 16 + 4 * h) = eb;
+			if (k == 0 && wave == 0) *(int32_t*)(lds2 + wF + (NWK + 1) * 16 + 8 + 4 * h) = fa;
 		};
 		const bool forecast = NWK < 24 ? (s_new == 64 || s_new == 256 || s_new == 1024) : NWK >= 64 ? (s_new == 1024 || s_new == 4096) : false;
 		int32_t far = kDeadPair;
@@ -539,13 +553,13 @@
 
 			const int32_t E1a = e1h[P1][k][0], E1b = e1h[P1][k][1], F1a = f1h[P1][k][0], F1b = f1h[P1][k][1];
 			const int32_t E2a = e2h[P2][k][0], E2b = e2h[P2][k][1], F2a = f2h[P2][k][0], F2b = f2h[P2][k][1];
-			const int32_t o1mA = FOLD ? 0 : left_of_A(O1.y, N1), o2mA = left_of_A(O2.y, N2), g1mA = left_of_A(E1b, xE1), g2mA = left_of_A(E2b, xE2);
-			const int32_t o1pB = FOLD ? 0 : right_of_B(O1.x, N1), o2pB = right_of_B(O2.x, N2), g1pB = right_of_B(F1a, xF1), g2pB = right_of_B(F2a, xF2);
+			const int32_t o1mA = FOLD ? 0 : left_of_A(O1.y, N1), o2mA = kFold2 ? 0 : left_of_A(O2.y, N2), g1mA = left_of_A(E1b, xE1), g2mA = left_of_A(E2b, xE2);
+			const int32_t o1pB = FOLD ? 0 : right_of_B(O1.x, N1), o2pB = kFold2 ? 0 : right_of_B(O2.x, N2), g1pB = right_of_B(F1a, xF1), g2pB = right_of_B(F2a, xF2);
 			const int32_t ONE = 0x00010001;
-			int32_t ne1A = FOLD ? g1mA : pk_max(o1mA, g1mA), ne2A = pk_max(o2mA, g2mA);
-			int32_t ne1B = FOLD ? E1a : pk_max(O1.x, E1a), ne2B = pk_max(O2.x, E2a);
-			const int32_t pf1A = FOLD ? F1b : pk_max(O1.y, F1b), pf2A = pk_max(O2.y, F2b);
-			const int32_t pf1B = FOLD ? g1pB : pk_max(o1pB, g1pB), pf2B = pk_max(o2pB, g2pB);
+			int32_t ne1A = FOLD ? g1mA : pk_max(o1mA, g1mA), ne2A = kFold2 ? g2mA : pk_max(o2mA, g2mA);
+			int32_t ne1B = FOLD ? E1a : pk_max(O1.x, E1a), ne2B = kFold2 ? E2a : pk_max(O2.x, E2a);
+			const int32_t pf1A = FOLD ? F1b : pk_max(O1.y, F1b), pf2A = kFold2 ? F2b : pk_max(O2.y, F2b);
+			const int32_t pf1B = FOLD ? g1pB : pk_max(o1pB, g1pB), pf2B = kFold2 ? g2pB : pk_max(o2pB, g2pB);
 			int32_t nf1A = pk_add(pf1A, ONE), nf2A = pk_add(pf2A, ONE), nf1B = pk_add(pf1B, ONE), nf2B = pk_add(pf2B, ONE);
 			const int32_t mA = pk_add(HX.x, ONE), mB = pk_add(HX.y, ONE);
 			int32_t hA, hB;
@@ -633,7 +647,7 @@
 				}
 			}
 			e1h[P1][k][0] = ne1A, e1h[P1][k][1] = ne1B, f1h[P1][k][0] = nf1A, f1h[P1][k][1] = nf1B;
-			e2h[P2][k][0] = ne2A, e2h[P2][k][1] = ne2B, f2h[P2][k][0] = nf2A, f2h[P2][k][1] = nf2B;
+			if (!kFold2) e2h[P2][k][0] = ne2A, e2h[P2][k][1] = ne2B, f2h[P2][k][0] = nf2A, f2h[P2][k][1] = nf2B;
 #pragma unroll
 			for (int i = 0; i < 2; ++i) {
 #pragma unroll
@@ -647,7 +661,8 @@
 					asm volatile("v_swap_b32 %0, %1" : "+v"(f2h[a - 1][k][i]), "+v"(f2h[a][k][i]));
 				}
 			}
-			put_edge(k, ne1B, ne2B, nf1A, nf2A);
+			if (kFold2) put_edge_half(k, 0, ne1B, nf1A);
+			else put_edge(k, ne1B, ne2B, nf1A, nf2A);
 
 #if MWF_B2_TIMING == 2
 			if (timed) asm volatile("s_memtime %0\n\ts_waitcnt lgkmcnt(0)" : "=s"(tc2) : "v"(hA), "v"(hB), "v"(rjA), "v"(dA) : "memory");
@@ -713,6 +728,13 @@
 			int32_t cA = MWF_BC(int32_t, (us2_t)__builtin_amdgcn_cvt_pk_u16((uint32_t)cnt[0], (uint32_t)cnt[2]));
 			int32_t cB = MWF_BC(int32_t, (us2_t)__builtin_amdgcn_cvt_pk_u16((uint32_t)cnt[1], (uint32_t)cnt[3]));
 			if (TAB) cA = MWF_BC(int32_t, (us2_t)(MWF_BC(us2_t, cA) >> 1)), cB = MWF_BC(int32_t, (us2_t)(MWF_BC(us2_t, cB) >> 1));
+			if (kFold2) {
+				int32_t px = O2.x, py = O2.y;
+				asm volatile("" : "+v"(px), "+v"(py));
+				ne2A = pk_max(ne2A, px), ne2B = pk_max(ne2B, py), nf2A = pk_max(nf2A, px), nf2B = pk_max(nf2B, py);
+				e2h[P2][k][0] = ne2A, e2h[P2][k][1] = ne2B, f2h[P2][k][0] = nf2A, f2h[P2][k][1] = nf2B;
+				put_edge_half(k, 1, ne2B, nf2A);
+			}
 #if MWF_B2_TIMING == 2
 			if (timed) asm volatile("s_memtime %0\n\ts_waitcnt lgkmcnt(0)" : "=s"(tc3) : "v"(cA), "v"(cB) : "memory");
 #endif
@@ -1000,6 +1022,7 @@
 		else
 			fprintf(stderr, "[libmwf_hip] band2 launch: T %d K %d E1 %d E2 %d TB %d S2 %d BI4 %d FOLD %d, %d pairs, grid %d\n", T, K, E1, E2, (int)TB, (int)S2, (int)BI4, (int)FOLD, (int)a.n_pairs, grid);
 		if (kTabProbe) fprintf(stderr, "[libmwf_hip] band2 table probe: table %d B, lds %d B\n", (int)a.band_lds_tab, lds);
+		if (kFold2Form) fprintf(stderr, "[libmwf_hip] band2 second fold: wfa_band2_tab2_kernel, row of lag %d folded one penalty ahead (o2 + e2 %d, bound %d)\n", (int)(a.pen.oe2 - a.pen.e2), (int)a.pen.oe2, kFold2MaxLag);
 	}
 	hipLaunchKernelGGL((MWF_BAND2_KERNEL<T, K, E1, E2, TB, S2, BI4, FOLD>), dim3(grid), dim3(T), lds, st, a);
 }
@@ -1033,8 +1056,13 @@
 	BatchArgs a = a0;
 	a.band_lds_seq = lds_seq, a.band_lds_tab = lds_tab;
 	const int lds = lds_seq + lds_tail<T, K, E1, E2>();
-	if (a.want_cigar) launch_variant<T, K, E1, E2, true, S2, BI4>(a, grid, lds, st);
-	else launch_variant<T, K, E1, E2, false, S2, BI4>(a, grid, lds, st);
+	if constexpr (kFold2Form) {
+		if (a.want_cigar) return -1;
+		launch_variant<T, K, E1, E2, false, S2, BI4>(a, grid, lds, st);
+	} else {
+		if (a.want_cigar) launch_variant<T, K, E1, E2, true, S2, BI4>(a, grid, lds, st);
+		else launch_variant<T, K, E1, E2, false, S2, BI4>(a, grid, lds, st);
+	}
 	return hipGetLastError() == hipSuccess ? 0 : -2;
 }
 
@@ -1044,9 +1072,10 @@
 	constexpr bool S2 = band2_geo_seq2(T);
 	if (seq2 != S2) return 0;
 	const int lds = lds_seq + lds_tail<T, K, E1, E2>();
-	return tb ? occ_variant<T, K, E1, E2, true, S2, BI4>(lds) : occ_variant<T, K, E1, E2, false, S2, BI4>(lds);
-}
-
-}
-
-}
+	if constexpr (kFold2Form) return tb ? 0 : occ_variant<T, K, E1, E2, false, S2, BI4>(lds);
+	else return tb ? occ_variant<T, K, E1, E2, true, S2, BI4>(lds) : occ_variant<T, K, E1, E2, false, S2, BI4>(lds);
+}
+
+}
+
+}
diff --git a/miniwfa_amd/csrc/mwf_band2_tab2.hip b/miniwfa_amd/csrc/mwf_band2_tab2.hip
--- /dev/null
+++ b/miniwfa_amd/csrc/mwf_band2_tab2.hip
@@ -0,0 +1,35 @@
+#define MWF_BAND2_FORM 3
+#include "mwf_band2_dispatch.h"
+
+namespace mwf {
+
+namespace {
+struct Unit {
+	using Sets = Tab2Sets;
+	using BiasedSets = NoSets;
+	static constexpr unsigned geos = kGeoWide;
+};
+bool tab2_geom_ok(const Penalty &p, const BandGeom &g)
+{
+	return g.packed == 1 && g.block == 512 && g.seq2 != 0 && g.tab > 0 && g.tab % 16 == 0 && g.lds_bytes > g.tab && g.fold2 != 0 && band2_tab2_supported(p);
+}
+}
+
+bool band2_tab2_supported(const Penalty &p)
+{
+	return has_pen_set(Unit::Sets{}, p.e1, p.e2) && band2_folds(p, true) && p.e2 == 1 && p.oe2 - p.e2 >= 3 && p.oe2 <= kFold2MaxLag;
+}
+
+int launch_band2_tab2(const BatchArgs &a, int grid, const BandGeom &g, void *stream)
+{
+	if (!tab2_geom_ok(a.pen, g) || !a.band_fold || a.want_cigar) return -1;
+	return band2_unit_launch<Unit>(a, grid, g, stream);
+}
+
+int band2_occupancy_tab2(const Penalty &p, const BandGeom &g, bool cigar)
+{
+	if (!tab2_geom_ok(p, g) || cigar) return 0;
+	return band2_unit_occupancy<Unit>(p, g, cigar);
+}
+
+}
diff --git a/miniwfa_amd/csrc/mwf_engine.cpp b/miniwfa_amd/csrc/mwf_engine.cpp
--- a/miniwfa_amd/csrc/mwf_engine.cpp
+++ b/miniwfa_amd/csrc/mwf_engine.cpp
@@ -78,6 +78,7 @@
 	else if (!strcmp(name, "dev_retry")) g->dev_retry = value != 0;
 	else if (!strcmp(name, "band_fold")) g->band_fold = value != 0;
 	else if (!strcmp(name, "probe_table")) g->probe_table = value != 0;
+	else if (!strcmp(name, "band_fold2")) g->band_fold2 = value != 0;
 	else if (!strcmp(name, "alpha_remap") && (value == 0 || value == 1)) g->alpha_remap = (int)value;
 	else if (!strcmp(name, "alpha16") && (value == 0 || value == 1)) g->alpha16 = (int)value;
 	else if (!strcmp(name, "trim")) { (void)hipSetDevice(g->device); trim(g); }
diff --git a/miniwfa_amd/csrc/mwf_engine.h b/miniwfa_amd/csrc/mwf_engine.h
--- a/miniwfa_amd/csrc/mwf_engine.h
+++ b/miniwfa_amd/csrc/mwf_engine.h
@@ -48,10 +48,10 @@
 	int kind = 0, block = 0;
 	bool ext = false;
 	int packed = 0, lane = 0, slots512 = 0, e1 = 0, e2 = 0, lds_bytes = 0;
-	bool cigar = false, seq2 = false, tab = false, nib = false;
+	bool cigar = false, seq2 = false, tab = false, nib = false, fold2 = false;
 	bool stream_pass = false, ring16 = false, big_ring = false;
 	int lds_e2_cols = 0;
-	auto tied() const { return std::tie(kind, block, ext, packed, lane, slots512, e1, e2, lds_bytes, cigar, seq2, tab, nib, stream_pass, ring16, big_ring, lds_e2_cols); }
+	auto tied() const { return std::tie(kind, block, ext, packed, lane, slots512, e1, e2, lds_bytes, cigar, seq2, tab, nib, fold2, stream_pass, ring16, big_ring, lds_e2_cols); }
 	bool operator<(const OccKey &o) const { return tied() < o.tied(); }
 };
 
@@ -74,6 +74,7 @@
 	bool dev_retry = true;
 	bool band_fold = true;
 	bool probe_table = true;
+	bool band_fold2 = true;
 	int64_t probe_table_lds = 0;
 	bool div_aware = true;
 	int64_t tun_gen = 0;
diff --git a/miniwfa_amd/csrc/mwf_internal.h b/miniwfa_amd/csrc/mwf_internal.h
--- a/miniwfa_amd/csrc/mwf_internal.h
+++ b/miniwfa_amd/csrc/mwf_internal.h
@@ -184,6 +184,7 @@
 	int lane;
 	int tab;
 	int nib;
+	int fold2 = 0;
 };
 bool coop_supported(const Penalty &p);
 int64_t coop_chunk_slots(int grid);
@@ -219,6 +220,7 @@
 int  launch_band2_bi2(const BatchArgs &a, int grid, const BandGeom &g, void *stream);
 int  launch_band2_tab(const BatchArgs &a, int grid, const BandGeom &g, void *stream);
 int  launch_band2_nib(const BatchArgs &a, int grid, const BandGeom &g, void *stream);
+int  launch_band2_tab2(const BatchArgs &a, int grid, const BandGeom &g, void *stream);
 int  band2_occupancy_e3(const Penalty &p, const BandGeom &g, bool cigar);
 int  band2_occupancy_e4(const Penalty &p, const BandGeom &g, bool cigar);
 int  band2_occupancy_bi1(const Penalty &p, const BandGeom &g, bool cigar);
@@ -227,6 +229,8 @@
 int  band2_occupancy_nib(const Penalty &p, const BandGeom &g, bool cigar);
 bool band2_nib_supported(const Penalty &p);
 bool band2_tab_supported(const Penalty &p, bool band_fold);
+int  band2_occupancy_tab2(const Penalty &p, const BandGeom &g, bool cigar);
+bool band2_tab2_supported(const Penalty &p);
 bool band2_biased512_supported(const Penalty &p);
 int  band2_biased512_chunks();
 int  band2_span_chunks();
diff --git a/miniwfa_amd/csrc/mwf_plan.cpp b/miniwfa_amd/csrc/mwf_plan.cpp
--- a/miniwfa_amd/csrc/mwf_plan.cpp
+++ b/miniwfa_amd/csrc/mwf_plan.cpp
@@ -152,6 +152,7 @@
 		if (tab + bg.lds_bytes <= budget) {
 			pl.band.tab = (int)tab, pl.band.lds_bytes = (int)(tab + bg.lds_bytes);
 			pl.cigar = (opt.flag & MWF_F_CIGAR) != 0;
+			pl.band.fold2 = (!pl.cigar && g->band_fold2 && band2_tab2_supported(P)) ? 1 : 0;
 			if (cached_occupancy(g, P, pl, 0, false) < 2) pl.band = bg;
 		}
 	}
@@ -163,7 +164,7 @@
 	if (pl.kind == 3) key.kind = 3, key.block = pl.block, key.ext = pl.ext;
 	else if (pl.kind == 2) {
 		key.kind = 2, key.block = pl.band.block, key.packed = pl.band.packed, key.lane = pl.band.lane, key.slots512 = pl.band.block == 512 ? pl.band.span / 2048 : 0;
-		key.e1 = P.e1, key.e2 = P.e2, key.lds_bytes = pl.band.lds_bytes, key.cigar = pl.cigar, key.seq2 = pl.band.seq2 != 0, key.tab = pl.band.tab > 0, key.nib = pl.band.nib != 0;
+		key.e1 = P.e1, key.e2 = P.e2, key.lds_bytes = pl.band.lds_bytes, key.cigar = pl.cigar, key.seq2 = pl.band.seq2 != 0, key.tab = pl.band.tab > 0, key.nib = pl.band.nib != 0, key.fold2 = pl.band.fold2 != 0;
 	} else key.block = pl.block, key.stream_pass = stream_pass, key.ring16 = ring16, key.big_ring = P.nH > kMaxRing, key.lds_e2_cols = lds_e2_cols;
 	auto it = g->occ_cache.find(key);
 	if (it != g->occ_cache.end()) return it->second;
```
